# antoni-wojcik/OpenCL-Raytracing

Hardware: AMD Instinct MI355X
Metric: Msamples/sec (rays/sec) at 1920×1080, 64 spp; % HBM roofline (higher is better)
Workload: dtype f32

## Files before the change

include/rt_amd.h:

```cpp
#ifndef RT_AMD_H
#define RT_AMD_H

#include <stddef.h>
#include <stdint.h>

#ifdef __cplusplus
extern "C" {
#endif

#define RT_ABI_VERSION 3

#define RT_OK 0
#define RT_EINVAL (-1)
#define RT_ENODEVICE (-2)
#define RT_EHIP (-3)
#define RT_ESTATE (-4)
#define RT_ERANGE (-5)

#define RT_TRIANGLE_EPSILON 0.0000001f
#define RT_MIN_DISTANCE 0.001f
#define RT_MAX_DISTANCE 1000.0f
#define RT_DEPTH 30
#define RT_RANDOM_BUFFER_SIZE 100000
#define RT_RANDOM_TABLE_FLOATS (4 * RT_RANDOM_BUFFER_SIZE)
// ... 290 lines not shown
int rt_read_variance(rt_context *ctx, int which, float *out, size_t bytes);
int rt_device_variance(rt_context *ctx, int which, void **d_out);

#define RT_DENOISE_MOMENTS_MIN_COUNT 4u
int rt_read_moments(rt_context *ctx, float *m2, size_t bytes);
int rt_device_moments(rt_context *ctx, void **d_m2);
int rt_moments_merge(uint32_t nA, const float sumA[3], float m2A, uint32_t nB, const float sumB[3], float m2B, float *m2_out);
int rt_denoise_moments(rt_context *ctx, const rt_denoise_variance_params *p);

int rt_sync(rt_context *ctx);

int rt_trace_samples(rt_context *ctx, const float camera[12], const uint32_t *x, const uint32_t *y,
                     const uint32_t *sample, size_t n, float *out_rgb);


int rt_read_image(rt_context *ctx, float *rgba, size_t bytes);

int rt_read_linear(rt_context *ctx, float *rgba, size_t bytes);

int rt_device_image(rt_context *ctx, void **d_rgba);
int rt_device_accum(rt_context *ctx, void **d_rgba);

#define RT_OPT_PREFIX_SHARING 1
#define RT_OPT_MAX_THREADS_PER_LAUNCH 2
#define RT_OPT_SAMPLE_QUEUE 3
#define RT_OPT_ACCEL 4
#define RT_OPT_WALK_SLICES 5
#define RT_OPT_PREFIX_TREE 7
#define RT_OPT_WAVE_FILL 8
#define RT_OPT_PREFIX_CACHE 9
#define RT_OPT_LOOKAHEAD 10
#define RT_OPT_EXACT_GRID 11
#define RT_OPT_MOMENTS 12
#define RT_OPT_ARITH 6
#define RT_ARITH_IEEE 0
#define RT_ARITH_ROCM_OCL_NOCONTRACT 1
#define RT_ARITH_ROCM_OCL 2
int rt_set_option(rt_context *ctx, int option, int value);


int rt_enable_counters(rt_context *ctx, int enable);
int rt_reset_counters(rt_context *ctx);
int rt_get_counters(rt_context *ctx, rt_counters *out);

int rt_debug_check_accel(const rt_scene_desc *scene, uint64_t stats[8], char *err, size_t err_len);

int rt_get_debug_counters(rt_context *ctx, uint64_t out[2]);

int rt_walk_overflow(rt_context *ctx, uint32_t *flags_out);

uint64_t rt_counters_bytes(const rt_counters *c);

int rt_last_kernel_ms(rt_context *ctx, float *ms);

int rt_kernel_ms_history(rt_context *ctx, float *ms, size_t cap, size_t *n_out);

int rt_debug_hit(rt_context *ctx, int kind, const float *rays, const uint32_t *prim, const uint32_t *face, size_t n,
                 float *out12);
int rt_debug_material(rt_context *ctx, int routine, const float *in16, size_t n, float *out9);
int rt_debug_div3(rt_context *ctx, const float *in4, size_t n, float *out6);
int rt_debug_builtin(rt_context *ctx, int op, const float *in8, size_t n, float *out4);
int rt_debug_queue_sums(rt_context *ctx, const float *in3, uint32_t npix, uint32_t count, uint32_t group_log2, float *out4);

int rt_stage_ms_history(rt_context *ctx, float *first_ms, float *second_ms, size_t cap, size_t *n_out);

int rt_prefix_cache_stats(rt_context *ctx, uint64_t *hits, uint64_t *misses);

int rt_lookahead_stats(rt_context *ctx, uint64_t *batches, uint64_t *served, uint64_t *direct, uint64_t *discarded);

int rt_lookahead_plan(int width, int height, int option_value, uint32_t sample_counter, uint32_t *batch_out);

int rt_sample_units(uint32_t seg_cap, uint32_t pixels_per_unit, uint32_t count_light, uint32_t count_heavy, uint32_t *units_out);

int rt_sample_grid_stats(rt_context *ctx, uint64_t *launches, uint64_t *exact, uint64_t *workgroups, uint64_t *live_last);

int rt_debug_live_list(rt_context *ctx, uint32_t out[4]);

int rt_debug_queue_pixels(uint32_t count, uint32_t waves_per_simd, uint32_t static_float4, uint32_t granule, uint32_t *pixels_out);

typedef struct rt_sample_facts {
    uint32_t count, glog2;
    uint32_t n, seg_cap;
    uint32_t material_count, sphere_count, plane_count, lens_count, model_count;
    uint32_t sphere_bvh, mesh_bvh;
    uint32_t walk_jobs;
    uint32_t faces;
    uint32_t cu_count;
    uint32_t count_enabled, sample_queue, walk_slices, wave_fill, moments;
    uint32_t exact, count_light, count_heavy;
} rt_sample_facts;

#define RT_PLAN_FIXED 0u
#define RT_PLAN_QUEUE 1u
#define RT_PLAN_WALK 2u
#define RT_PLAN_GENERIC_COUNT 0xFFFFFFFFu

typedef struct rt_sample_plan {
    uint32_t family;
    uint32_t count, accel, geom, waves, moments, count_log2, multi;
// ... 50 lines not shown
```

opencl-raytracing_amd/_abi.py:

```python
import ctypes as C

import numpy as np

RT_ABI_VERSION = 3
DEPTH = 30
RANDOM_BUFFER_SIZE = 100000
RANDOM_TABLE_FLOATS = 4 * RANDOM_BUFFER_SIZE
MAX_DIM = 16384
MAX_SAMPLE = 65535

T_REFRACTIVE, T_REFLECTIVE, T_DIELECTRIC, T_DIFFUSE, T_TEXTURED, T_LIGHT = range(6)
MAT_NAMES = {
    "refractive": T_REFRACTIVE,
    "reflective": T_REFLECTIVE,
    "dielectric": T_DIELECTRIC,
    "diffuse": T_DIFFUSE,
    "textured": T_TEXTURED,
    "light": T_LIGHT,
}

MATERIAL = np.dtype([("type", "<i4"), ("_p0", "<i4", (3,)), ("color", "<f4", (4,)), ("extra_data", "<f4"),
                     ("_p1", "<i4", (3,))])
SPHERE = np.dtype([("pos", "<f4", (4,)), ("r", "<f4"), ("mat_ID", "<u4"), ("_p", "<u4", (2,))])
PLANE = np.dtype([("pos", "<f4", (4,)), ("normal", "<f4", (4,)), ("mat_ID", "<u4"), ("_p", "<u4", (3,))])
# ... 118 lines not shown
    _fields_ = [("iterations", C.c_uint32), ("sigma_luminance", C.c_float), ("sigma_normal", C.c_float),
                ("sigma_position", C.c_float), ("sigma_albedo", C.c_float), ("flags", C.c_uint32)]


def denoise_prototypes(lib):
    vp, sz = C.c_void_p, C.c_size_t
    lib.rt_render_features.argtypes = [vp, vp]
    lib.rt_read_features.argtypes = [vp, vp, sz]
    lib.rt_device_features.argtypes = [vp, C.POINTER(vp)]
    lib.rt_denoise.argtypes = [vp, C.POINTER(DenoiseParams)]
    lib.rt_read_denoised.argtypes = [vp, vp, sz]
    lib.rt_device_denoised.argtypes = [vp, C.POINTER(vp)]
    lib.rt_denoise_variance.argtypes = [vp, C.POINTER(DenoiseVarianceParams)]
    lib.rt_read_variance.argtypes = [vp, C.c_int, vp, sz]
    lib.rt_device_variance.argtypes = [vp, C.c_int, C.POINTER(vp)]
    lib.rt_render_features_chain.argtypes = [vp, vp, C.POINTER(FeatureChainParams)]
    lib.rt_feature_chain_signature.argtypes = [vp, C.c_uint32, C.POINTER(C.c_uint32)]


DENOISE_MOMENTS_MIN_COUNT = 4


def moments_prototypes(lib):
    vp, sz, u32, f32 = C.c_void_p, C.c_size_t, C.c_uint32, C.c_float
    f3 = C.POINTER(f32)
    lib.rt_read_moments.argtypes = [vp, vp, sz]
    lib.rt_device_moments.argtypes = [vp, C.POINTER(vp)]
    lib.rt_moments_merge.argtypes = [u32, f3, f32, u32, f3, f32, f3]
    lib.rt_denoise_moments.argtypes = [vp, C.POINTER(DenoiseVarianceParams)]


def prefix_cache_prototypes(lib):
    lib.rt_prefix_cache_stats.argtypes = [C.c_void_p, C.POINTER(C.c_uint64), C.POINTER(C.c_uint64)]


def lookahead_prototypes(lib):
    p64 = C.POINTER(C.c_uint64)
    lib.rt_lookahead_stats.argtypes = [C.c_void_p, p64, p64, p64, p64]
    lib.rt_lookahead_plan.argtypes = [C.c_int, C.c_int, C.c_int, C.c_uint32, C.POINTER(C.c_uint32)]


def sample_grid_prototypes(lib):
    p64, u32 = C.POINTER(C.c_uint64), C.c_uint32
    lib.rt_sample_units.argtypes = [u32, u32, u32, u32, C.POINTER(u32)]
    lib.rt_sample_grid_stats.argtypes = [C.c_void_p, p64, p64, p64, p64]
    lib.rt_debug_live_list.argtypes = [C.c_void_p, C.POINTER(u32)]
    lib.rt_debug_wave_fixed.argtypes = [C.c_void_p, C.POINTER(C.c_uint64)]
    lib.rt_debug_stage_block.argtypes = [C.c_void_p, C.c_void_p, C.c_size_t, C.POINTER(u32)]
    lib.rt_debug_queue_pixels.argtypes = [u32, u32, u32, u32, C.POINTER(u32)]
    lib.rt_debug_queue_occupancy.argtypes = [C.c_void_p, u32, C.POINTER(C.c_int)]
    lib.rt_debug_plan_samples.argtypes = [C.POINTER(SampleFacts), C.POINTER(SamplePlan)]
    lib.rt_debug_last_sample_plan.argtypes = [C.c_void_p, C.POINTER(SampleFacts), C.POINTER(SamplePlan)]


class _U32Record(C.Structure):

    def __init__(self, **kw):
        super().__init__(**{k: int(v) for k, v in kw.items()})

    def as_dict(self):
        return {k: int(getattr(self, k)) for k, _ in self._fields_}


class SampleFacts(_U32Record):
    _fields_ = [(k, C.c_uint32) for k in (
        "count", "glog2", "n", "seg_cap", "material_count", "sphere_count", "plane_count", "lens_count", "model_count",
# ... 289 lines not shown
```

opencl-raytracing_amd/csrc/pt_kernels.hip:

```cpp
#include <hip/hip_runtime.h>

#include <algorithm>

#include "pt_device.hpp"
#include "pt_moments.hpp"
#include "pt_chain.hpp"
#include "rt_context.hpp"
#include "pt_kernels.hpp"

#ifndef PT_GATHER_UNIT
#define PT_GATHER_UNIT 0
#endif

namespace PT_NS {
using namespace rtamd;


PT_DEV uint32_t live_take(const FrameParams &fp, const uint32_t *__restrict__ live_count, uint32_t unit, uint32_t want,
                          uint32_t &first) {
    const uint32_t cap = fp.seg_cap;
    const uint32_t cnt_l = min(live_count[0], cap);
    const uint32_t cnt_h = min(live_count[LIVE_HEAVY_COUNTER], cap - cnt_l);
    const uint32_t units_h = want ? (cnt_h + want - 1u) / want : 0u;
    const bool heavy = unit < units_h;
// ... 12 lines not shown
    for (int i = 0; i < PT_N_COUNTERS; i++) {
        uint32_t v = cn.c[i];
#pragma unroll
        for (int off = 32; off > 0; off >>= 1) v += __shfl_xor(v, off);
        if ((threadIdx.x & 63) == 0 && v) atomicAdd(&row[i], (unsigned long long)v * scale);
    }
}

PT_DEV void zero_counters(LaneCounters &cn) {
#pragma unroll
    for (int i = 0; i < PT_N_COUNTERS; i++) cn.c[i] = 0;
}

PT_DEV uint32_t lanes_below(unsigned long long m) {
    return __builtin_amdgcn_mbcnt_hi((uint32_t)(m >> 32), __builtin_amdgcn_mbcnt_lo((uint32_t)m, 0u));
}

PT_DEV V3 group_sum(V3 sum, uint32_t g) {
    for (uint32_t off = g >> 1; off > 0; off >>= 1) {
        sum.x += __shfl_xor(sum.x, off);
        sum.y += __shfl_xor(sum.y, off);
        sum.z += __shfl_xor(sum.z, off);
    }
    return sum;
}

PT_DEV void accumulate(float4 *__restrict__ accum, size_t pix, V3 sum, uint32_t count) {
    float4 a = accum[pix];
    a.x += sum.x;
    a.y += sum.y;
    a.z += sum.z;
    a.w += (float)count;
    accum[pix] = a;
}

PT_DEV void moments_update(const float4 *accum, float *m2, size_t pix, V3 sum, uint32_t count, float m2B) {
    const float4 a = accum[pix];
    m2[pix] = moments_merge(a.w, a.x, a.y, a.z, m2[pix], (float)count, sum.x, sum.y, sum.z, m2B);
}

struct LaneMoments {
    float n, m2;
};
PT_DEV void moments_fold(LaneMoments &lm, V3 sum, V3 s) {
    lm.m2 = moments_merge(lm.n, sum.x, sum.y, sum.z, lm.m2, 1.0f, s.x, s.y, s.z, 0.0f);
    lm.n += 1.0f;
}
PT_DEV V3 group_sum_moments(V3 sum, LaneMoments &lm, uint32_t g) {
    for (uint32_t off = g >> 1; off > 0; off >>= 1) {
        const V3 o = mk(__shfl_xor(sum.x, off), __shfl_xor(sum.y, off), __shfl_xor(sum.z, off));
        const float on = __shfl_xor(lm.n, off), om2 = __shfl_xor(lm.m2, off);
        lm.m2 = moments_merge(lm.n, sum.x, sum.y, sum.z, lm.m2, on, o.x, o.y, o.z, om2);
        lm.n += on;
        sum.x += o.x;
        sum.y += o.y;
        sum.z += o.z;
    }
    return sum;
}

PT_DEV V3 final_sum(V3 col, uint32_t count, uint32_t group_log2) {
    const uint32_t g = 1u << group_log2;
    V3 Y = mk(0.0f, 0.0f, 0.0f);
    for (uint32_t k = 0; k < (count >> group_log2); k++) Y = Y + col;
    V3 X = Y + col;
    uint32_t r = count & (g - 1u);
// ... 178 lines not shown

#ifndef PT_PREFIX_WAVES
#define PT_PREFIX_WAVES 4
#endif
template <bool COUNT, bool ACCEL, bool TREES = false>
__global__ __launch_bounds__(256, TREES ? PT_PREFIX_WAVES : 1) void pt_prefix(DeviceScene sc, FrameParams fp, PixelRec *__restrict__ recs,
                                                 uint32_t *__restrict__ live, uint32_t *__restrict__ live_count,
                                                 float4 *__restrict__ accum, unsigned long long *counters,
                                                 FinalPix *__restrict__ finals, uint32_t *__restrict__ final_n) {
    __shared__ float4 s_mat[PT_LDS_STATIC_FLOAT4];
    LaneCounters cn;
    if (COUNT) zero_counters(cn);
    Ctx c{sc, stage_materials(sc, s_mat), &cn};
    c.lwin = staged_winners(sc, s_mat);
    c.lpln = staged_planes(sc, s_mat);

    uint32_t slot = fp.slot_begin + blockIdx.x * 256u + threadIdx.x;
    uint32_t x = 0, y = 0;
    bool valid = slot < fp.slot_end && slot_to_pixel(fp, slot, x, y) && pixel_active(fp, x, y);
    bool is_live = false, is_final = false;
    PixelRec rec;
    rec.p_kind = rec.n_extra = rec.d = rec.out = rec.col = make_float4(0.0f, 0.0f, 0.0f, 0.0f);
    if (valid) {
        Ray r0 = primary_ray(fp.cam, x, y, fp.w, fp.h);
        rec = trace_prefix<COUNT, ACCEL>(c, r0, x, y);
    }
    if (valid) {
        bool final_px = (__float_as_uint(rec.p_kind.w) & 0xFFu) == REC_FINAL;
        if (final_px) {
            is_final = true;
            if (accum) {
                const V3 fsum = final_sum(xyz(rec.out), fp.count, fp.group_log2);
                if (fp.m2) moments_update(accum, fp.m2, (size_t)y * fp.w + x, fsum, fp.count, 0.0f);
                accumulate(accum, (size_t)y * fp.w + x, fsum, fp.count);
            }
            if (COUNT) cn.c[CN_SAMPLES] += 1;
        } else {
            is_live = true;
        }
    }
    const uint32_t lane = threadIdx.x & 63u, wv = threadIdx.x >> 6;
    const uint32_t kb = __float_as_uint(rec.p_kind.w);
    const bool lane_heavy = valid && (((kb >> 8) & 0xFFu) >= 2u || is_glass_vertex(rec));
    const bool wg_heavy = __syncthreads_or(lane_heavy ? 1 : 0) != 0;
    const bool glass = TREES && is_live && is_glass_vertex(rec);
    __shared__ uint32_t s_wave_n[4], s_wave_g[4], s_wave_f[4], s_base, s_tree0;
    __shared__ uint32_t s_tpos[256];
    __shared__ uint32_t s_wn[PT_TREE_LEVELS];
    __shared__ uint16_t s_wait[PT_TREE_LEVELS > 2 ? 2 : 1][256u << (PT_TREE_LEVELS - 1)];
    unsigned long long m = __ballot(is_live);
    const unsigned long long gm = __ballot(glass);
    const unsigned long long fm = __ballot(is_final);
    if (lane == 0) {
        s_wave_n[wv] = (uint32_t)__popcll(m);
        s_wave_f[wv] = (uint32_t)__popcll(fm);
        if (TREES) s_wave_g[wv] = (uint32_t)__popcll(gm);
    }
    __syncthreads();
    if (threadIdx.x == 0) {
        uint32_t total = s_wave_n[0] + s_wave_n[1] + s_wave_n[2] + s_wave_n[3];
        s_base = total ? atomicAdd(&live_count[wg_heavy ? LIVE_HEAVY_COUNTER : 0u], total) : 0u;
        if (TREES) {
            const uint32_t trees = s_wave_g[0] + s_wave_g[1] + s_wave_g[2] + s_wave_g[3];
            s_tree0 = trees ? atomicAdd(fp.tree_count, trees) : 0u;
            for (uint32_t l = 0; l < PT_TREE_LEVELS; l++) s_wn[l] = 0u;
        }
    }
// ... 27 lines not shown
        uint32_t before = 0;
        for (uint32_t k = 0; k < wv; k++) before += s_wave_g[k];
        const uint32_t j = before + lanes_below(gm);
        if (j < nt) {
            s_tpos[j] = pos;
            fp.trees[tree0 + j].dec[0].hsh = 0u;
        }
    }
    __syncthreads();
    for (uint32_t level = 0; level < PT_TREE_LEVELS; level++) {
        const uint32_t items = 2u * (level ? s_wn[level] : nt);
        for (uint32_t t = threadIdx.x; t < items; t += 256u) {
            const uint32_t e = level ? (uint32_t)s_wait[(level - 1u) & 1u][t >> 1] : (1u << 8) | (t >> 1);
            const uint32_t j = e & 0xFFu, heap = e >> 8, which = t & 1u, tree = tree0 + j;
            if (tree_step<ACCEL>(c, fp.trees + tree, tree, heap, which, level + 1u == PT_TREE_LEVELS, recs + s_tpos[j],
                                 fp.tree_wait + (size_t)tree * PT_TREE_WAITS)) {
                const uint32_t k = atomicAdd(&s_wn[level + 1u], 1u);
                s_wait[level & 1u][k] = (uint16_t)(((2u * heap + which) << 8) | j);
            }
        }
        if (level + 1u < PT_TREE_LEVELS) __syncthreads();
    }
}

#if !PT_GATHER_UNIT
__global__ __launch_bounds__(256) void pt_final_replay(FrameParams fp, const FinalPix *__restrict__ finals,
                                                       const uint32_t *__restrict__ final_n, float4 *__restrict__ accum) {
    if (threadIdx.x >= min(final_n[blockIdx.x], 256u)) return;
    const FinalPix e = finals[blockIdx.x * 256u + threadIdx.x];
    uint32_t x = 0, y = 0;
    if (!slot_to_pixel(fp, e.slot, x, y)) return;
    const V3 fsum = final_sum(mk(e.r, e.g, e.b), fp.count, fp.group_log2);
    if (fp.m2) moments_update(accum, fp.m2, (size_t)y * fp.w + x, fsum, fp.count, 0.0f);
    accumulate(accum, (size_t)y * fp.w + x, fsum, fp.count);
}
#endif

PT_DEV size_t ring_at(const FrameParams &fp, size_t pix, uint32_t j) {
    return PT_RING_PIXEL_MAJOR ? pix * fp.count + j : j * ((size_t)fp.w * fp.h) + pix;
}

#if !PT_GATHER_UNIT
__global__ __launch_bounds__(256) void pt_final_retrace(FrameParams fp, const FinalPix *__restrict__ finals,
                                                        const uint32_t *__restrict__ final_n) {
    if (threadIdx.x >= min(final_n[blockIdx.x], 256u)) return;
    const FinalPix e = finals[blockIdx.x * 256u + threadIdx.x];
    uint32_t x = 0, y = 0;
    if (!slot_to_pixel(fp, e.slot, x, y)) return;
    const size_t pix = (size_t)y * fp.w + x;
    const float4 at = fp.la_image[pix];
    V3 prev = mk(at.x, at.y, at.z);
    const V3 sum = mk(0.0f, 0.0f, 0.0f) + mk(e.r, e.g, e.b);
    for (uint32_t j = 0; j < fp.count; j++) {
        prev = retrace_step(prev, sum, fp.first + j);
        fp.la_ring[ring_at(fp, pix, j)] = make_float4(prev.x, prev.y, prev.z, 1.0f);
    }
}
#endif

template <bool COUNT, bool ACCEL>
__global__ __launch_bounds__(256) void pt_samples(DeviceScene sc, FrameParams fp, const PixelRec *__restrict__ recs,
                                                  const uint32_t *__restrict__ live,
                                                  const uint32_t *__restrict__ live_count,
                                                  float4 *__restrict__ accum, unsigned long long *counters) {
    __shared__ float4 s_mat[PT_LDS_STATIC_FLOAT4];
    {
        uint32_t e0 = 0;
// ... 214 lines not shown
    q.slot[3 * idx + 2] = rgb.z;
}

#ifndef PT_QUEUE_SUMS_TREE
#define PT_QUEUE_SUMS_TREE 1
#endif
PT_DEV V3 queue_lane_sum(const WaveQueue &q, uint32_t p, uint32_t l, uint32_t g) {
    V3 sum = mk(0.0f, 0.0f, 0.0f);
    const uint32_t n = p < q.npix ? q.count : 0u;
    for (uint32_t j = l; j < n; j += g) {
        const LdsF32 sl = q.slot + 3u * (p * q.count + j);
        sum = sum + mk(sl[0], sl[1], sl[2]);
    }
    return sum;
}
template <int OFF>
PT_DEV float row_add(float v) {
    return v + __int_as_float(__builtin_amdgcn_update_dpp(0, __float_as_int(v), 0x100 + OFF, 0xF, 0xF, false));
}
template <int OFF>
PT_DEV V3 row_add(V3 v) { return mk(row_add<OFF>(v.x), row_add<OFF>(v.y), row_add<OFF>(v.z)); }
PT_DEV float row_pair_add(float a, float b) {
    const auto r = __builtin_amdgcn_permlane16_swap(__float_as_uint(a), __float_as_uint(b), false, false);
    return __uint_as_float(r[0]) + __uint_as_float(r[1]);
}
PT_DEV V3 queue_lane_slot64(const WaveQueue &q, uint32_t p, uint32_t l) {
    V3 sum = mk(0.0f, 0.0f, 0.0f);
    if (p < q.npix) {
        const LdsF32 sl = q.slot + 3u * (p * 64u + l);
        sum = sum + mk(sl[0], sl[1], sl[2]);
    }
    return sum;
}
template <int CL = -1>
PT_DEV void queue_sums_tree(const WaveQueue &q, const FrameParams &fp, float4 *__restrict__ accum) {
    if (CL == 6) {
        static_assert(QUEUE_SLOTS / 64u <= 8u, "two passes of four pixels");
        const uint32_t lane = threadIdx.x, half = lane >> 5, i = lane & 31u, row = lane >> 4;
#pragma unroll
        for (uint32_t pb = 0; pb < 8u; pb += 4u) {
            if (pb >= q.npix) break;
            V3 a = queue_lane_slot64(q, pb + half, i), b = queue_lane_slot64(q, pb + 2u + half, i);
            a = a + queue_lane_slot64(q, pb + half, i + 32u);
            b = b + queue_lane_slot64(q, pb + 2u + half, i + 32u);
            V3 sum = mk(row_pair_add(a.x, b.x), row_pair_add(a.y, b.y), row_pair_add(a.z, b.z));
            sum = row_add<1>(row_add<2>(row_add<4>(row_add<8>(sum))));
            const uint32_t p = pb + ((row & 1u) << 1 | row >> 1);
            if (p < q.npix && (lane & 15u) == 0u) accumulate(accum, (size_t)q.xy[p].y * fp.w + q.xy[p].x, sum, 64u);
        }
        return;
    }
    const uint32_t lane = threadIdx.x, gl = fp.group_log2;
    if (gl >= 5u) {
        const uint32_t half = lane >> 5, i = lane & 31u, g = 1u << gl, row = lane >> 4;
        for (uint32_t pb = 0; pb < q.npix; pb += 4u) {
            V3 a = queue_lane_sum(q, pb + half, i, g), b = queue_lane_sum(q, pb + 2u + half, i, g);
            if (gl == 6u) {
                a = a + queue_lane_sum(q, pb + half, i + 32u, g);
                b = b + queue_lane_sum(q, pb + 2u + half, i + 32u, g);
            }
            V3 sum = mk(row_pair_add(a.x, b.x), row_pair_add(a.y, b.y), row_pair_add(a.z, b.z));
            sum = row_add<1>(row_add<2>(row_add<4>(row_add<8>(sum))));
            const uint32_t p = pb + ((row & 1u) << 1 | row >> 1);
            if (p < q.npix && (lane & 15u) == 0u) accumulate(accum, (size_t)q.xy[p].y * fp.w + q.xy[p].x, sum, q.count);
        }
    } else {
        const uint32_t g = 1u << gl, ppp = 64u >> gl;
        for (uint32_t pb = 0; pb < q.npix; pb += ppp) {
            const uint32_t p = pb + (lane >> gl), l = lane & (g - 1u);
            V3 sum = queue_lane_sum(q, p, l, g);
            if (gl >= 4u) sum = row_add<8>(sum);
            if (gl >= 3u) sum = row_add<4>(sum);
            if (gl >= 2u) sum = row_add<2>(sum);
            if (gl >= 1u) sum = row_add<1>(sum);
            if (p < q.npix && l == 0u) accumulate(accum, (size_t)q.xy[p].y * fp.w + q.xy[p].x, sum, q.count);
        }
    }
}
template <bool MOMENTS, bool BUTTERFLY = false, int CL = -1>
PT_DEV void queue_sums(const WaveQueue &q, const FrameParams &fp, float4 *__restrict__ accum) {
    __builtin_amdgcn_fence(__ATOMIC_SEQ_CST, "wavefront");
    __builtin_amdgcn_wave_barrier();
    if (PT_QUEUE_SUMS_TREE && !MOMENTS && !BUTTERFLY) return queue_sums_tree<CL>(q, fp, accum);
    const uint32_t lane = threadIdx.x;
    const uint32_t g = 1u << fp.group_log2, ppp = 64u >> fp.group_log2;
    for (uint32_t pb = 0; pb < q.npix; pb += ppp) {
        uint32_t p = pb + (lane >> fp.group_log2), l = lane & (g - 1u);
        V3 sum = mk(0.0f, 0.0f, 0.0f);
        if (p < q.npix)
            for (uint32_t j = l; j < q.count; j += g) {
                const LdsF32 sl = q.slot + 3u * (p * q.count + j);
                sum = sum + mk(sl[0], sl[1], sl[2]);
            }
        sum = group_sum(sum, g);
        if (MOMENTS) {
            const float mean = moments_lum(sum.x, sum.y, sum.z) / (float)q.count;
            float dev2 = 0.0f;
            if (p < q.npix)
                for (uint32_t j = l; j < q.count; j += g) {
                    const LdsF32 sl = q.slot + 3u * (p * q.count + j);
                    const float d = moments_lum(sl[0], sl[1], sl[2]) - mean;
                    dev2 += d * d;
                }
            for (uint32_t off = g >> 1; off > 0; off >>= 1) dev2 += __shfl_xor(dev2, off);
            if (p < q.npix && l == 0) moments_update(accum, fp.m2, (size_t)q.xy[p].y * fp.w + q.xy[p].x, sum, q.count, dev2);
        }
        if (p < q.npix && l == 0) accumulate(accum, (size_t)q.xy[p].y * fp.w + q.xy[p].x, sum, q.count);
    }
}

static_assert(QUEUE_MAX_PIXELS * 4u <= 64u, "queue_replay maps (pixel, channel) to the wave's lanes");
template <bool CAM = false>
PT_DEV void queue_replay(const WaveQueue &q, const FrameParams &fp) {
    static_assert(!CAM || !PT_RING_PIXEL_MAJOR, "the camera look-ahead's start image is frame 0 of a frame-major ring (one contiguous "
                                                "device copy of the image); the pixel-major A/B layout has no such frame");
    __builtin_amdgcn_fence(__ATOMIC_SEQ_CST, "wavefront");
// ... 842 lines not shown
static_assert(MODE_ACCUM == 0 && MODE_TRACE == 1 && MODE_RETRACE == 2, "render_kernel's table is indexed by the mode");
static RenderKernel render_kernel(int mode, bool count, bool accel) {
    static const RenderKernel k[3][2][2] = {
        {{pt_render<MODE_ACCUM, false, false>, pt_render<MODE_ACCUM, false, true>}, {pt_render<MODE_ACCUM, true, false>, pt_render<MODE_ACCUM, true, true>}},
        {{pt_render<MODE_TRACE, false, false>, pt_render<MODE_TRACE, false, true>}, {pt_render<MODE_TRACE, true, false>, pt_render<MODE_TRACE, true, true>}},
        {{pt_render<MODE_RETRACE, false, false>, pt_render<MODE_RETRACE, false, true>}, {pt_render<MODE_RETRACE, true, false>, pt_render<MODE_RETRACE, true, true>}}};
    return k[mode][count][accel];
}

static uint32_t slots_per_launch(const rt_context *ctx, uint32_t glog2) { return std::max(ctx->max_threads_per_launch >> glog2, 1u); }
static uint32_t range_end(uint32_t b, uint32_t slots, uint32_t per) { return slots - b > per ? b + per : slots; }

template <class Body>
static int launch_ranges(rt_context *ctx, FrameParams &fp, uint32_t slots, Body body) {
    const uint32_t per = slots_per_launch(ctx, fp.group_log2);
    hipEvent_t *evp = ctx->ev[ctx->ev_count % rt_context::EV_RING];
    HIP_TRY(ctx, hipEventRecord(evp[0], ctx->stream));
    HIP_TRY(ctx, hipEventRecord(evp[2], ctx->stream));
    for (uint32_t b = 0; b < slots; b = fp.slot_end) {
        fp.slot_begin = b;
        fp.slot_end = range_end(b, slots, per);
        const int rc = body();
        if (rc != RT_OK) return rc;
    }
    HIP_TRY(ctx, hipGetLastError());
    HIP_TRY(ctx, hipEventRecord(evp[1], ctx->stream));
    ctx->ev_count++;
    return RT_OK;
}

int launch_render(rt_context *ctx, int mode, const float cam[12], uint32_t first, uint32_t count, uint32_t glog2, float4 *accum,
                  const BlockMask *mask, float *m2) {
    if (mode < MODE_ACCUM || mode > MODE_RETRACE) return fail(ctx, RT_EINVAL, "unknown render mode %d", mode);
    FrameParams fp = frame_params(ctx, cam, first, count, glog2);
    apply_mask(fp, mask);
    fp.m2 = mode == MODE_ACCUM ? m2 : nullptr;
    const DeviceScene sc = device_scene(ctx);
    const uint32_t slots = fp.slot_end;
    if (slots == 0) return RT_OK;
    const RenderKernel kernel = render_kernel(mode, ctx->count_enabled, scene_has_accel(sc));
    return launch_ranges(ctx, fp, slots, [&]() -> int {
        const uint64_t threads = (uint64_t)(fp.slot_end - fp.slot_begin) << glog2;
        hipLaunchKernelGGL(kernel, dim3((unsigned)((threads + 255) / 256)), dim3(256), 0, ctx->stream, sc, fp, accum, ctx->image.p, ctx->counters.p);
        return RT_OK;
    });
}

using SampleFacts = rt_sample_facts;
using SamplePlan = rt_sample_plan;
using CameraFacts = rt_camera_facts;
using CameraPlan = rt_camera_plan;

struct QueueSize {
    uint32_t accel, geom, waves, pixels_per_wave, ppw_cap, lds_face_f4, static_f4, lds_bytes;
};
template <class Facts>
static QueueSize queue_size(const Facts &f, bool stage_faces) {
    QueueSize q = {};
    const bool simple_geom = f.lens_count == 0 && f.model_count == 0;
    const bool sphere_bvh_only = f.sphere_bvh && !f.mesh_bvh;
    q.accel = f.sphere_bvh || f.mesh_bvh;
    q.geom = !q.accel || sphere_bvh_only ? (simple_geom ? 0u : 1u) : 2u;
    q.waves = !q.accel ? PT_Q_WAVES : ((sphere_bvh_only && simple_geom) ? PT_Q_WAVES_SPHERE_BVH : PT_Q_WAVES_ACCEL);
    q.static_f4 = lds_static_used(f.material_count, f.sphere_count, f.plane_count);
    const uint32_t want_units = (f.cu_count ? f.cu_count : 256u) * 4u * 6u * PT_UNITS_PER_WAVE_SLOT;
    const uint32_t ppw_full = (64u + f.count - 1u) / f.count;
// ... 140 lines not shown
}

using PrefixKernel = void (*)(DeviceScene, FrameParams, PixelRec *, uint32_t *, uint32_t *, float4 *, unsigned long long *, FinalPix *, uint32_t *);
static PrefixKernel prefix_kernel(bool count, bool accel, bool trees) {
    static const PrefixKernel plain[2][2] = {{pt_prefix<false, false>, pt_prefix<false, true>}, {pt_prefix<true, false>, pt_prefix<true, true>}};
    static const PrefixKernel tree[2] = {pt_prefix<false, false, true>, pt_prefix<false, true, true>};
    return trees ? tree[accel] : plain[count][accel];
}
static void launch_first_stage(rt_context *ctx, const DeviceScene &sc, const FrameParams &fp, bool hit, bool lookahead, float4 *accum, uint32_t *live_count) {
    const rt_context::Slots &ss = ctx->slots;
    const dim3 grid(fp.seg_cap / 256u), block(256);
    if (!hit)
        hipLaunchKernelGGL(prefix_kernel(ctx->count_enabled, scene_has_accel(sc), fp.tree_cap != 0u), grid, block, 0, ctx->stream, sc, fp,
                           ss.recs.p, ss.live.p, live_count, accum, ctx->counters.p, ss.finals.p, ss.final_n.p);
    else if (!lookahead)
        hipLaunchKernelGGL(pt_final_replay, grid, block, 0, ctx->stream, fp, ss.finals.p, ss.final_n.p, accum);
    if (lookahead) hipLaunchKernelGGL(pt_final_retrace, grid, block, 0, ctx->stream, fp, ss.finals.p, ss.final_n.p);
}

static bool lookahead_ok(const rt_context *ctx, const FrameParams &fp, const float4 *accum, const BlockMask *mask, const float *m2) {
    return !accum && !m2 && !mask && !ctx->count_enabled && ctx->world == 1 && ctx->sample_queue && fp.count <= QUEUE_SLOTS &&
           (ctx->max_threads_per_launch >> fp.group_log2) >= fp.slot_end;
}

static void refresh_stage_block(rt_context *ctx, const DeviceScene &sc) {
    if (!PT_STAGE_COPY || ctx->stage_block.generation == ctx->prefix_cache.generation) return;
    if (lds_static_used(sc.material_count, sc.sphere_count, sc.plane_count))
        hipLaunchKernelGGL(pt_stage_block, dim3(1), dim3(64), 0, ctx->stream, sc,
                           reinterpret_cast<float4 *>(reinterpret_cast<char *>(ctx->materials.p) + stage_block_offset(sc.material_count)));
    ctx->stage_block.generation = ctx->prefix_cache.generation;
    ctx->stage_block.builds++;
}

static int launch_fused_any(rt_context *ctx, const float cam[12], uint32_t first, uint32_t count, uint32_t glog2, float4 *accum,
                            const BlockMask *mask, float4 *ring, float *m2) {
    FrameParams fp = frame_params(ctx, cam, first, count, glog2);
    apply_mask(fp, mask);
    fp.m2 = m2;
    if (ring) {
        if (!lookahead_ok(ctx, fp, accum, mask, m2))
            return fail(ctx, RT_EINVAL, "a look-ahead launch needs the sample queue, an unsharded frame in one slot range and no counters");
        fp.la_ring = ring;
        fp.la_image = ctx->image.p;
    }
    const DeviceScene sc = device_scene(ctx);
    const uint32_t slots = fp.slot_end;
    if (slots == 0) return RT_OK;
    int rc = ensure_slots(ctx, slots);
    if (rc) return rc;
    refresh_stage_block(ctx, sc);
    const rt_context::Slots &ss = ctx->slots;
    uint32_t *live_count = ss.live.p + ss.capacity + 256u;
    const uint32_t per = slots_per_launch(ctx, glog2);
    const bool tree_on = ctx->prefix_tree == 2 || (ctx->prefix_tree == 1 && count >= PT_TREE_MIN_SAMPLES);
    const bool keepable = !mask && !ctx->count_enabled && per >= slots;
    uint32_t cam_bits[12];
    memcpy(cam_bits, cam, sizeof cam_bits);
    const bool hit = prefix_lookup(ctx->prefix_cache, keepable, tree_on, cam_bits);
    bool exact = false;
    if ((rc = learn_live_counts(ctx, hit, live_count, &exact)) != RT_OK) return rc;
    rt_context::SampleGrid &sg = ctx->sample_grid;
    hipEvent_t *evp = ctx->ev[ctx->ev_count % rt_context::EV_RING];
    HIP_TRY(ctx, hipEventRecord(evp[0], ctx->stream));
    for (uint32_t b = 0; b < slots; b = fp.slot_end) {
        fp.slot_begin = b;
        fp.slot_end = range_end(b, slots, per);
        if (!hit) HIP_TRY(ctx, hipMemsetAsync(live_count, 0, LIVE_COUNT_STRIDE * sizeof(uint32_t), ctx->stream));
        fp.trees = ss.trees.p;
        fp.tree_wait = ss.tree_wait.p;
        fp.tree_count = live_count + LIVE_TREE_COUNTER;
        fp.tree_cap = (tree_on && !ctx->count_enabled) ? (uint32_t)ss.tree_capacity : 0u;
        fp.seg_cap = (fp.slot_end - fp.slot_begin + 255u) / 256u * 256u;
        const SampleFacts facts = sample_facts(ctx, sc, fp, exact);
        const SamplePlan plan = plan_samples(facts);
        fp.lds_face_f4 = plan.lds_face_f4;
        launch_first_stage(ctx, sc, fp, hit, ring != nullptr, accum, live_count);
        HIP_TRY(ctx, hipEventRecord(evp[2], ctx->stream));
        if ((rc = launch_plan(ctx, plan, sc, fp, accum, live_count)) != RT_OK) return rc;
        sg.last_facts = facts, sg.last_plan = plan;
        sg.launches++;
        sg.workgroups += plan.grid_units;
        if (plan.grid_units && plan.family == RT_PLAN_QUEUE && plan.count_log2 == 6u) sg.count64_launches++;
        if (exact) { sg.exact_launches++; sg.live_last = plan.grid_units; }
    }
    HIP_TRY(ctx, hipGetLastError());
    HIP_TRY(ctx, hipEventRecord(evp[1], ctx->stream));
    ctx->ev_count++;
    if (hit) ctx->prefix_cache.hits++; else ctx->prefix_cache.misses++;
    if (keepable) prefix_keep(ctx->prefix_cache, tree_on, cam_bits);
    return RT_OK;
}

int launch_fused(rt_context *ctx, const float cam[12], uint32_t first, uint32_t count, uint32_t glog2, float4 *accum, const BlockMask *mask, float *m2) {
    return launch_fused_any(ctx, cam, first, count, glog2, accum, mask, nullptr, m2);
}

int launch_lookahead(rt_context *ctx, const float cam[12], uint32_t first, uint32_t count, float4 *ring) {
    if (!ring || count < 1u) return fail(ctx, RT_EINVAL, "look-ahead launch without a ring");
    return launch_fused_any(ctx, cam, first, count, group_log2_for(count), nullptr, nullptr, ring, nullptr);
}

static RenderKernel camera_render_kernel(bool count, bool accel) {
    static const RenderKernel k[2][2] = {{pt_render<MODE_ACCUM, false, false, true>, pt_render<MODE_ACCUM, false, true, true>},
                                         {pt_render<MODE_ACCUM, true, false, true>, pt_render<MODE_ACCUM, true, true, true>}};
    return k[count][accel];
}
typedef void (*RayRenderKernel)(DeviceScene, FrameParams, float4 *, unsigned long long *);
static RayRenderKernel ray_render_kernel(bool count, bool accel, bool sets) {
    static const RayRenderKernel k[2][2] = {{pt_render_rays<false, false>, pt_render_rays<false, true>},
                                            {pt_render_rays<true, false>, pt_render_rays<true, true>}};
    static const RayRenderKernel k_sets[2][2] = {{pt_render_raysets<false, false>, pt_render_raysets<false, true>},
// ... 1 lines not shown
    return sets ? k_sets[count][accel] : k[count][accel];
}
static const pt::GatherKernels &gather_kernels() {
#if PT_ARITH == 0
    return *pt::gather_kernels_a0();
#elif PT_ARITH == 1
    return *pt::gather_kernels_a1();
#else
    return *pt::gather_kernels_a2();
#endif
}

struct SampleSource {
    bool rays, hemi;
    const void *p;
    size_t n;
    uint32_t set_size;
    const float *cam0;
};

static int launch_source(rt_context *ctx, const SampleSource &src, uint32_t first, uint32_t count, uint32_t glog2, float4 *accum,
                         const BlockMask *mask, float *m2, float4 *ring) {
    const bool sets = src.set_size != 0u && !src.hemi;
    if (!src.rays) {
        if (!src.p || count < 1u || count > RT_SPP_PER_LAUNCH) return fail(ctx, RT_EINVAL, "a camera launch takes 1 .. %u blocks", RT_SPP_PER_LAUNCH);
    } else {
        if (!src.p || !accum || src.n < 1u || src.n > (1u << 28) || count < 1u || count > RT_SPP_PER_LAUNCH)
            return fail(ctx, RT_EINVAL, "a ray launch takes 1 .. 2^28 rays and 1 .. %u samples", RT_SPP_PER_LAUNCH);
        if (src.set_size > RT_RAY_SET_MAX || (uint64_t)src.n * src.set_size > (1ull << 31))
            return fail(ctx, RT_EINVAL, "a ray-set launch takes sets of 1 .. %u records, 2^31 records in all", RT_RAY_SET_MAX);
        if (mask && src.n != (size_t)ctx->width * ctx->height)
            return fail(ctx, RT_EINVAL, "a masked ray launch takes one ray per pixel of the %d x %d frame", ctx->width, ctx->height);
    }
    FrameParams fp = src.rays ? frame_params(ctx, src.cam0, first, count, glog2, 0, 1)
                              : frame_params(ctx, src.cam0, first, count, glog2);
    apply_mask(fp, mask);
    fp.m2 = m2;
    if (src.rays) fp.rays = reinterpret_cast<const float4 *>(src.p);
    else fp.cams = reinterpret_cast<const float *>(src.p);
    const DeviceScene sc = device_scene(ctx);
    if (ring) {
        if (src.rays || !lookahead_ok(ctx, fp, accum, mask, m2) || plan_camera_samples(camera_facts(ctx, sc, fp)).family != RT_CAMERA_PLAN_QUEUE)
            return fail(ctx, RT_EINVAL, "a look-ahead launch needs the sample queue, an unsharded frame in one slot range and no counters");
        fp.la_ring = ring;
    }
    const uint32_t slots = src.rays ? (uint32_t)src.n : fp.slot_end;
    if (slots == 0) return RT_OK;
    refresh_stage_block(ctx, sc);
    return launch_ranges(ctx, fp, slots, [&]() -> int {
        const CameraFacts facts = camera_facts(ctx, sc, fp);
        const CameraPlan plan = plan_camera_samples(facts);
        const dim3 grid(plan.grid_units), block(plan.block_size);
        fp.lds_face_f4 = plan.lds_face_f4;
        if (plan.family == RT_CAMERA_PLAN_QUEUE) {
            const QueueRow *r = find_queue_row(ctx, src.rays ? "ray" : "camera", plan.accel, plan.geom, plan.waves);
            if (!r) return RT_ESTATE;
            const QueueKernel kernel = !src.rays ? r->cams[ring != nullptr] : src.hemi ? gather_kernels().queue(plan.accel, plan.geom, plan.waves)
                                       : sets ? r->ray_sets : r->rays;
            if (!kernel) return fail(ctx, RT_ESTATE, "no pt_samples_q_hemi for the plan (accel %u, geom %u, %u waves)", plan.accel, plan.geom, plan.waves);
            hipLaunchKernelGGL(kernel, grid, block, plan.lds_bytes, ctx->stream,
                               sc, fp, (const PixelRec *)nullptr, (const uint32_t *)nullptr, (const uint32_t *)nullptr, accum,
                               ctx->counters.p, plan.pixels_per_wave);
        } else if (src.rays) {
            hipLaunchKernelGGL(src.hemi ? gather_kernels().fixed(plan.count != 0u, plan.accel != 0u) : ray_render_kernel(plan.count != 0u, plan.accel != 0u, sets),
                               grid, block, 0, ctx->stream, sc, fp, accum, ctx->counters.p);
        } else {
// ... 218 lines not shown
```

opencl-raytracing_amd/csrc/pt_samples_q_kernel.hpp:

```cpp
#if PT_Q_LOOKAHEAD_FORM == 4
template <bool ACCEL, int GEOM, int WAVES>
__global__ __launch_bounds__(64, WAVES) void pt_samples_q_hemi(DeviceScene sc, FrameParams fp, const PixelRec *__restrict__ recs,
                                                         const uint32_t *__restrict__ live,
                                                         const uint32_t *__restrict__ live_count,
                                                         float4 *__restrict__ accum, unsigned long long *counters,
                                                         uint32_t pixels_per_wave) {
    constexpr bool COUNT = false, MOMENTS = false, CAM = true, CAM_LA = false, RAYS = true, SETS = false, HEMI = true;
    constexpr int COUNT_LOG2 = -1;
#elif PT_Q_LOOKAHEAD_FORM == 3
template <bool ACCEL, int GEOM, int WAVES>
__global__ __launch_bounds__(64, WAVES) void pt_samples_q_raysets(DeviceScene sc, FrameParams fp, const PixelRec *__restrict__ recs,
                                                            const uint32_t *__restrict__ live,
                                                            const uint32_t *__restrict__ live_count,
                                                            float4 *__restrict__ accum, unsigned long long *counters,
                                                            uint32_t pixels_per_wave) {
    constexpr bool COUNT = false, MOMENTS = false, CAM = true, CAM_LA = false, RAYS = true, SETS = true, HEMI = false;
    constexpr int COUNT_LOG2 = -1;
#elif PT_Q_LOOKAHEAD_FORM == 2
template <bool ACCEL, int GEOM, int WAVES>
__global__ __launch_bounds__(64, WAVES) void pt_samples_q_rays(DeviceScene sc, FrameParams fp, const PixelRec *__restrict__ recs,
                                                         const uint32_t *__restrict__ live,
                                                         const uint32_t *__restrict__ live_count,
                                                         float4 *__restrict__ accum, unsigned long long *counters,
                                                         uint32_t pixels_per_wave) {
// ... 181 lines not shown
                hn = h.n;
                hmat = h.mat;
                int type;
                float extra;
                load_material<BY_COUNT>(c, h.mat, type, extra, col);
                if (BY_USE) htype = (uint32_t)type;
                if (type == RT_LIGHT) {
                    if (SIP_HIT) out = vmin<MIN_FAST>(out, col);
                    else res = vmin<MIN_FAST>(out, col);
                    done = true;
                } else if (type == RT_TEXTURED) {
                    if (COUNT) cn.c[CN_N_TEXFETCH]++;
                    float tu = h.u, tv = h.v;
                    if (PT_TEXEL_LAZY && GEOM == 0 && !COUNT && !ACCEL) asm("" : "+v"(tu), "+v"(tv));
                    col = texture_rgb(c.sc, tu, tv, h.tex);
                }
            }
            if (done) {
                queue_put(q, idx, SIP_HIT ? out : res);
                active = false;
            } else if (PT_RNG_PREFETCH == 2) {
                rnd = fetch_rnd_b(sc.table, r.d, depth, bv, bu);
            }
        }
        PT_STAMP(c, 4);
    }
#if PT_STAMPS
    if (threadIdx.x == 0 && q.npix)
        for (int k = 0; k < 6; k++) atomicAdd(&counters[(size_t)COUNTER_REPLICAS * COUNTER_STRIDE + k], c.st[k]);
#endif
    static_assert(!CAM_LA || (CAM && ACCEL), "the look-ahead kernels of the camera entry's ACCEL rows");
    constexpr bool LA_BRANCH = CAM ? !ACCEL : !COUNT && !MOMENTS;
    if (CAM_LA || (!RAYS && LA_BRANCH && fp.la_ring)) queue_replay<CAM>(q, fp);
    else queue_sums<MOMENTS, COUNT || ACCEL, COUNT_LOG2>(q, fp, accum);
    flush_counters<COUNT>(cn, counters, 1);
}
```

opencl-raytracing_amd/csrc/pt_types.hpp:

```cpp
#pragma once
#include <hip/hip_runtime.h>
#include <stdint.h>

#include "../../include/rt_amd.h"

namespace pt {

#define PT_DEV __device__ __forceinline__
#define PT_HD __host__ __device__ inline

#define PT_LDS_MATERIALS 64
#define PT_LDS_WINNERS 64
#define PT_SPHERE_BATCH 4

struct DeviceScene {
    const rt_material *materials;
    const rt_sphere *spheres;
    const float4 *sph4;
    const rt_plane *planes;
    const rt_lens *lenses;
    const rt_float3 *vertices;
    const rt_float2 *uvs;
    const uint32_t *indices;
    const rt_mesh *meshes;
    const rt_model *models;
    const float *table;
    const float4 *tex;
    int tex_w, tex_h, tex_layers;
    float tex_wf, tex_hf;
    uint32_t material_count, sphere_count, sphere_batches, plane_count, lens_count, model_count;
    const float4 *faces;
    const uint32_t *mesh_face_base;
    const float4 *mbvh_nodes;
    const float4 *mbvh_faces;
// ... 51 lines not shown
#define PT_TREE_LEVELS 2
#endif
#define PT_TREE_DECISIONS ((1 << PT_TREE_LEVELS) - 1)
#define PT_TREE_LEAVES (1 << PT_TREE_LEVELS)
struct TreeDecision {
    uint32_t hsh;
    float prob;
    uint32_t depth;
    uint16_t child[2];
};
struct PixelTree {
    TreeDecision dec[PT_TREE_DECISIONS + 1];
    PixelRec leaf[PT_TREE_LEAVES];
};
#define PT_TREE_WAITS (PT_TREE_LEAVES - 2)

enum RenderMode { MODE_ACCUM = 0, MODE_TRACE = 1, MODE_RETRACE = 2 };

#ifndef PT_RING_PIXEL_MAJOR
#define PT_RING_PIXEL_MAJOR 0
#endif

struct FrameParams {
    float cam[12];
    int w, h;
    int tile_w_log2, tile_h_log2;
    uint32_t tiles_x, tiles_total;
    uint32_t rank, world;
    uint32_t slot_begin, slot_end;
    uint32_t first, count;
    uint32_t group_log2;
    uint32_t seg_cap;
    float inv_count;
    PixelTree *trees;
    PixelRec *tree_wait;
    uint32_t *tree_count;
    uint32_t tree_cap;
    uint32_t lds_face_f4;
    const uint32_t *block_active;
    uint32_t blk_w_log2, blk_h_log2, blocks_x;
    float4 *la_ring;
    union {
        const float4 *la_image;
        const float *cams;
        const float4 *rays;
        const float4 *feats;
    };
    float *m2;
};

struct BlockMask {
    const uint32_t *active;
    uint32_t w_log2, h_log2, blocks_x;
};

#define LIVE_COUNT_STRIDE 32u
#define LIVE_TREE_COUNTER 16u
#define LIVE_HEAVY_COUNTER 24u

#define COUNTER_REPLICAS 512
#define COUNTER_STRIDE 16

PT_DEV bool slot_to_pixel(const FrameParams &fp, uint32_t slot, uint32_t &x, uint32_t &y) {
    uint32_t tpix_log2 = fp.tile_w_log2 + fp.tile_h_log2;
    uint32_t k = slot >> tpix_log2, in = slot & ((1u << tpix_log2) - 1u);
    uint32_t t = fp.rank + k * fp.world;
    if (t >= fp.tiles_total) return false;
    uint32_t tx = t % fp.tiles_x, ty = t / fp.tiles_x;
    x = (tx << fp.tile_w_log2) + (in & ((1u << fp.tile_w_log2) - 1u));
    y = (ty << fp.tile_h_log2) + (in >> fp.tile_w_log2);
    return x < (uint32_t)fp.w && y < (uint32_t)fp.h;
}

PT_DEV bool pixel_active(const FrameParams &fp, uint32_t x, uint32_t y) {
    return !fp.block_active || fp.block_active[(y >> fp.blk_h_log2) * fp.blocks_x + (x >> fp.blk_w_log2)] != 0u;
}

PT_DEV bool ray_active(const FrameParams &fp, uint32_t index) {
    if (!fp.block_active) return true;
    const uint32_t y = index / (uint32_t)fp.w, x = index - y * (uint32_t)fp.w;
    return fp.block_active[(y >> fp.blk_h_log2) * fp.blocks_x + (x >> fp.blk_w_log2)] != 0u;
}
// ... 9 lines not shown
```

opencl-raytracing_amd/csrc/rt_amd.hip:

```cpp
#include <hip/hip_runtime.h>

#include <algorithm>
#include <cmath>
#include <cfloat>
#include <cstdarg>
#include <cstdio>
#include <cstdlib>
#include <cstring>
#include <functional>
#include <mutex>
#include <new>
#include <string>
#include <vector>

#include "rt_context.hpp"
#include "pt_kernels.hpp"
#include "pt_moments.hpp"
#include "pt_chain.hpp"
#include "scene_prep.hpp"

using namespace pt;
using namespace rtamd;
using namespace scene_prep;

// ... 236 lines not shown
    rt_context::Lookahead &la = ctx->lookahead;
    la.discarded += la.pending;
    la.pending = 0;
}

void lookahead_validate(rt_context *ctx) {
    const rt_context::Lookahead &la = ctx->lookahead;
    if (la.pending && (la.key_generation != ctx->prefix_cache.generation || la.key_epoch != ctx->image_epoch ||
                       la.next_sample != ctx->sample_counter + 1u))
        lookahead_drop(ctx);
}

int alloc_frame(rt_context *ctx, int w, int h) {
    ctx->slots = {};
    ctx->prefix_changed();
    ctx->image_epoch++;
    lookahead_drop(ctx);
    ctx->lookahead.ring = {};
    ctx->lookahead.ring_frames = 0;
    ctx->lookahead.ring_failed = false;
    ctx->adaptive = {};
    ctx->features = {};
    ctx->denoise = {};
    ctx->moments.m2 = {};
    ctx->moments.valid = false;
    const size_t px = (size_t)w * h;
    HIP_TRY(ctx, ctx->image.alloc(px));
    HIP_TRY(ctx, ctx->accum.alloc(px));
    HIP_TRY(ctx, hipMemset(ctx->image.p, 0, px * sizeof(float4)));
    HIP_TRY(ctx, hipMemset(ctx->accum.p, 0, px * sizeof(float4)));
    ctx->width = w;
    ctx->height = h;
    ctx->accum_count = 0;
    ctx->sample_counter = 0;
    return RT_OK;
}

int check_ready(rt_context *ctx, const float *cam) {
    if (!ctx) return RT_EINVAL;
    if (!cam) return fail(ctx, RT_EINVAL, "camera block is NULL");
    if (!ctx->have_scene) return fail(ctx, RT_ESTATE, "no scene: call rt_set_scene first");
    if (ctx->scene_uses_textures && (ctx->tex_layers <= 0 || ctx->max_texture_id >= (uint32_t)ctx->tex_layers))
        return fail(ctx, RT_ERANGE, "scene has textured meshes (max texture id %u) but only %d texture layers are set",
                    ctx->max_texture_id, ctx->tex_layers);
    return RT_OK;
}

}

namespace rtamd {
int read_back(rt_context *ctx, void *dst, size_t bytes, const void *src, size_t need, const char *what, bool ready,
              const char *producer) {
    if (!dst || bytes != need) return fail(ctx, RT_EINVAL, "%s buffer must be %zu bytes", what, need);
    if (!ready) return fail(ctx, RT_ESTATE, "no %s call since the frame was (re)allocated", producer);
    HIP_TRY(ctx, hipSetDevice(ctx->device));
    HIP_TRY(ctx, hipMemcpyAsync(dst, src, need, hipMemcpyDeviceToHost, ctx->stream));
    HIP_TRY(ctx, hipStreamSynchronize(ctx->stream));
    return RT_OK;
}
}

namespace {

int apply_arith(rt_context *ctx) {
    const bool w_is_radius = ctx->arith == RT_ARITH_ROCM_OCL;
    auto rec = [&](const rt_sphere &s) {
        volatile float r2 = s.r * s.r;
        return make_float4(s.pos.x, s.pos.y, s.pos.z, w_is_radius ? s.r : (float)r2);
    };
    const uint32_t n = (uint32_t)ctx->h_spheres.size();
    const uint32_t batches = (n + PT_SPHERE_BATCH - 1) / PT_SPHERE_BATCH;
    std::vector<float4> v((size_t)(batches + 1) * PT_SPHERE_BATCH, make_float4(0.0f, 0.0f, 0.0f, w_is_radius ? NAN : -INFINITY));
    for (uint32_t i = 0; i < n; i++) v[i] = rec(ctx->h_spheres[i]);
    HIP_TRY(ctx, ctx->sph4.upload(v.data(), v.size()));
    ctx->sphere_batches = batches;
    if (!ctx->h_bvh_idx.empty()) {
        std::vector<float4> leaf(ctx->h_bvh_idx.size());
        for (size_t i = 0; i < leaf.size(); i++) leaf[i] = rec(ctx->h_spheres[ctx->h_bvh_idx[i]]);
        HIP_TRY(ctx, ctx->bvh_sph.upload(leaf.data(), leaf.size()));
    }
    HIP_TRY(ctx, ctx->faces.upload(ctx->h_faces.data(), ctx->h_faces.size()));
    HIP_TRY(ctx, ctx->mbvh_faces.upload(ctx->h_mbvh_faces.data(), ctx->h_mbvh_faces.size()));
    if (ctx->arith != RT_ARITH_IEEE) {
        int rc = ctx->ks->launch_face_normals(ctx, ctx->faces.p, (uint32_t)(ctx->h_faces.size() / 3));
        if (rc == RT_OK) rc = ctx->ks->launch_face_normals(ctx, ctx->mbvh_faces.p, (uint32_t)(ctx->h_mbvh_faces.size() / 3));
        if (rc != RT_OK) return rc;
        HIP_TRY(ctx, hipStreamSynchronize(ctx->stream));
    }
    return RT_OK;
}

}


extern "C" {

int rt_abi_version(void) { return RT_ABI_VERSION; }

const char *rt_last_error(const rt_context *ctx) {
    if (ctx) return ctx->error.c_str();
    std::lock_guard<std::mutex> lk(g_err_mutex);
    return g_create_error.c_str();
}

int rt_make_random_table(uint64_t seed, float *out, size_t n) {
    if (!out || n != RT_RANDOM_TABLE_FLOATS) return fail(nullptr, RT_EINVAL, "table must hold %d floats", RT_RANDOM_TABLE_FLOATS);
    make_table(seed, out);
    return RT_OK;
}

int rt_create(int device, int width, int height, rt_context **out) {
    if (!out) return fail(nullptr, RT_EINVAL, "out is NULL");
    *out = nullptr;
    if (width < 1 || height < 1 || width > RT_MAX_DIM || height > RT_MAX_DIM)
        return fail(nullptr, RT_EINVAL, "frame size %dx%d outside 1..%d", width, height, RT_MAX_DIM);
    int n = 0;
    if (hipGetDeviceCount(&n) != hipSuccess || n < 1)
        return fail(nullptr, RT_ENODEVICE, "no HIP device visible (this library has no CPU path)");
    if (device < 0 || device >= n) return fail(nullptr, RT_ENODEVICE, "device %d out of range (%d visible)", device, n);
    hipDeviceProp_t prop;
// ... 30 lines not shown
    if (const char *e = getenv("RT_PREFIX_CACHE")) ctx->prefix_cache.enabled = strcmp(e, "0") != 0;
    if (const char *e = getenv("RT_LOOKAHEAD")) { if (strcmp(e, "0") == 0) ctx->lookahead.k = 0; }
    if (const char *e = getenv("RT_EXACT_GRID")) ctx->sample_grid.exact = strcmp(e, "0") != 0;
    if (hipHostMalloc((void **)&ctx->sample_grid.h_counts, LIVE_COUNT_STRIDE * sizeof(uint32_t), hipHostMallocDefault) != hipSuccess ||
        hipEventCreateWithFlags(&ctx->sample_grid.counts_ev, hipEventDisableTiming) != hipSuccess) { ctx->error = "live-count read-back allocation failed"; return bail(RT_EHIP); }
    if ((rc = alloc_frame(ctx, width, height)) != RT_OK) return bail(rc);
    if ((rc = rt_set_seed(ctx, 0xC0FFEEull)) != RT_OK) return bail(rc);
    if ((rc = rt_set_textures(ctx, nullptr, 0, 0, 0)) != RT_OK) return bail(rc);
    *out = ctx;
    return RT_OK;
}

void rt_destroy(rt_context *ctx) {
    if (!ctx) return;
    (void)hipSetDevice(ctx->device);
    if (ctx->own_stream) (void)hipStreamSynchronize(ctx->own_stream);
    for (int i = 0; i < rt_context::EV_RING; i++)
        for (int k = 0; k < 3; k++)
            if (ctx->ev[i][k]) (void)hipEventDestroy(ctx->ev[i][k]);
    if (ctx->sample_grid.counts_ev) (void)hipEventDestroy(ctx->sample_grid.counts_ev);
    if (ctx->sample_grid.h_counts) (void)hipHostFree(ctx->sample_grid.h_counts);
    for (hipEvent_t e : ctx->cameras.read)
        if (e) (void)hipEventDestroy(e);
    if (ctx->cameras.h_table) (void)hipHostFree(ctx->cameras.h_table);
    if (ctx->own_stream) (void)hipStreamDestroy(ctx->own_stream);
    delete ctx;
}

int rt_resize(rt_context *ctx, int width, int height) {
    if (!ctx) return RT_EINVAL;
    if (width < 1 || height < 1 || width > RT_MAX_DIM || height > RT_MAX_DIM)
        return fail(ctx, RT_EINVAL, "frame size %dx%d outside 1..%d", width, height, RT_MAX_DIM);
    HIP_TRY(ctx, hipSetDevice(ctx->device));
    HIP_TRY(ctx, hipStreamSynchronize(ctx->stream));
    return alloc_frame(ctx, width, height);
}

int rt_set_stream(rt_context *ctx, void *hip_stream) {
    if (!ctx) return RT_EINVAL;
    HIP_TRY(ctx, hipSetDevice(ctx->device));
    HIP_TRY(ctx, hipStreamSynchronize(ctx->stream));
    ctx->stream = hip_stream ? (hipStream_t)hip_stream : ctx->own_stream;
    ctx->prefix_changed();
    ctx->ev_count = 0;
    return RT_OK;
}

int rt_set_scene(rt_context *ctx, const rt_scene_desc *d) {
    if (!ctx) return RT_EINVAL;
    if (!d) return fail(ctx, RT_EINVAL, "scene is NULL");
    ctx->prefix_changed();
    {
        PreparedScene ps;
        std::string err;
        if (int rc = prepare_scene(*d, ps, err)) return fail(ctx, rc, "%s", err.c_str());
        HIP_TRY(ctx, hipSetDevice(ctx->device));
        HIP_TRY(ctx, hipStreamSynchronize(ctx->stream));
        ctx->have_scene = false;
        HIP_TRY(ctx, ctx->materials.upload(d->materials, d->material_count,
                                           lds_static_used(d->material_count, d->sphere_count, d->plane_count) * sizeof(float4)));
        ctx->stage_block.generation = ~0ull;
        HIP_TRY(ctx, ctx->spheres.upload(d->spheres, d->sphere_count));
        ctx->h_spheres.assign(d->spheres, d->spheres + d->sphere_count);
        HIP_TRY(ctx, ctx->mesh_face_base.upload(ps.face_base.data(), ps.face_base.size()));
        HIP_TRY(ctx, ctx->mbvh_nodes.upload(ps.mesh_packed.data(), ps.mesh_packed.size()));
        ctx->have_mesh_bvh = ps.have_mesh_bvh;
        HIP_TRY(ctx, ctx->mbvh_face_idx.upload(ps.leaf_face_idx.data(), ps.leaf_face_idx.size()));
        HIP_TRY(ctx, ctx->mesh_bvh_root.upload(ps.mesh_roots.data(), ps.mesh_roots.size()));
        ctx->walk_jobs.release();
        if (!ps.walk_jobs.empty()) HIP_TRY(ctx, ctx->walk_jobs.upload(ps.walk_jobs.data(), ps.walk_jobs.size()));
        ctx->bvh_node_count = ps.bvh_node_count;
        if (!ps.sphere_nodes.empty()) {
            HIP_TRY(ctx, ctx->bvh_nodes.upload(ps.sphere_boxes.data(), ps.sphere_boxes.size()));
            HIP_TRY(ctx, ctx->bvh_links.upload(ps.sphere_links.data(), ps.sphere_links.size()));
            HIP_TRY(ctx, ctx->bvh_idx.upload(ps.sphere_leaf_idx.data(), ps.sphere_leaf_idx.size()));
            ctx->bvh_rmax = ps.bvh_rmax;
            for (int k = 0; k < 3; k++) { ctx->bvh_lo[k] = ps.bvh_lo[k]; ctx->bvh_hi[k] = ps.bvh_hi[k]; }
        }
        HIP_TRY(ctx, ctx->planes.upload(d->planes, d->plane_count));
        HIP_TRY(ctx, ctx->lenses.upload(d->lenses, d->lens_count));
        HIP_TRY(ctx, ctx->vertices.upload(d->vertices, d->vertex_count));
        if (d->uv_count) HIP_TRY(ctx, ctx->uvs.upload(d->uvs, d->uv_count));
        else {
            std::vector<rt_float2> zeros(d->vertex_count ? d->vertex_count : 1, rt_float2{0.0f, 0.0f});
            HIP_TRY(ctx, ctx->uvs.upload(zeros.data(), d->vertex_count));
        }
        HIP_TRY(ctx, ctx->indices.upload(d->indices, d->index_count));
        HIP_TRY(ctx, ctx->meshes.upload(d->meshes, d->mesh_count));
        HIP_TRY(ctx, ctx->models.upload(d->models, d->model_count));
        ctx->scene_uses_textures = ps.uses_tex;
        ctx->max_texture_id = ps.max_tex;
        ctx->h_bvh_idx.swap(ps.sphere_leaf_idx);
        ctx->h_faces.swap(ps.faces);
        ctx->h_mbvh_faces.swap(ps.leaf_faces);
    }
    if (int rc = apply_arith(ctx)) return rc;
    ctx->have_scene = true;
    ctx->sample_counter = 0;
    return RT_OK;
}

int rt_set_textures(rt_context *ctx, const float *rgba, int w, int h, int layers) {
    if (!ctx) return RT_EINVAL;
    ctx->prefix_changed();
    HIP_TRY(ctx, hipSetDevice(ctx->device));
    HIP_TRY(ctx, hipStreamSynchronize(ctx->stream));
    if (layers == 0) {
        float4 zero = make_float4(0.0f, 0.0f, 0.0f, 0.0f);
        HIP_TRY(ctx, ctx->tex.upload(&zero, 1));
        ctx->tex_w = ctx->tex_h = 1;
        ctx->tex_layers = 0;
        return RT_OK;
    }
    if (!rgba || w < 1 || h < 1 || layers < 1 || w > 32768 || h > 32768 || layers > 2048)
        return fail(ctx, RT_EINVAL, "bad texture array %dx%dx%d", w, h, layers);
    HIP_TRY(ctx, ctx->tex.upload((const float4 *)rgba, (size_t)w * h * layers));
    ctx->tex_w = w;
    ctx->tex_h = h;
    ctx->tex_layers = layers;
    return RT_OK;
}

int rt_set_random_table(rt_context *ctx, const float *table, size_t n) {
    if (!ctx) return RT_EINVAL;
    if (!table || n != RT_RANDOM_TABLE_FLOATS) return fail(ctx, RT_EINVAL, "table must hold %d floats", RT_RANDOM_TABLE_FLOATS);
    ctx->prefix_changed();
    HIP_TRY(ctx, hipSetDevice(ctx->device));
    HIP_TRY(ctx, hipStreamSynchronize(ctx->stream));
    HIP_TRY(ctx, ctx->table.upload(table, n));
    return RT_OK;
}

int rt_set_seed(rt_context *ctx, uint64_t seed) {
    if (!ctx) return RT_EINVAL;
    std::vector<float> t(RT_RANDOM_TABLE_FLOATS);
    make_table(seed, t.data());
    return rt_set_random_table(ctx, t.data(), t.size());
}

int rt_get_random_table(rt_context *ctx, float *out, size_t n) {
    if (!ctx) return RT_EINVAL;
    if (!out || n != RT_RANDOM_TABLE_FLOATS) return fail(ctx, RT_EINVAL, "table must hold %d floats", RT_RANDOM_TABLE_FLOATS);
    HIP_TRY(ctx, hipSetDevice(ctx->device));
    HIP_TRY(ctx, hipStreamSynchronize(ctx->stream));
    HIP_TRY(ctx, hipMemcpy(out, ctx->table.p, n * sizeof(float), hipMemcpyDeviceToHost));
    return RT_OK;
}

int rt_set_shard(rt_context *ctx, int rank, int world, int tile_w, int tile_h) {
    if (!ctx) return RT_EINVAL;
    auto log2_exact = [](int v) { int l = 0; while ((1 << l) < v) l++; return (1 << l) == v ? l : -1; };
    int lw = log2_exact(tile_w), lh = log2_exact(tile_h);
    if (world < 1 || rank < 0 || rank >= world) return fail(ctx, RT_EINVAL, "rank %d of %d", rank, world);
    if (world > 1 && ctx->moments.on) return fail(ctx, RT_EINVAL, "RT_OPT_MOMENTS is 1: sample moments are kept on unsharded contexts only");
    if (tile_w < 1 || tile_h < 1 || lw < 0 || lh < 0 || lw + lh > 16)
        return fail(ctx, RT_EINVAL, "tile %dx%d: sides must be powers of two, area <= 65536", tile_w, tile_h);
    ctx->prefix_changed();
    ctx->rank = rank;
    ctx->world = world;
    ctx->tile_w_log2 = lw;
    ctx->tile_h_log2 = lh;
    return RT_OK;
}

extern "C++" {
namespace {

#if PT_RING_PIXEL_MAJOR
__global__ __launch_bounds__(256) void pt_ring_handout(const float4 *__restrict__ ring, float4 *__restrict__ image, size_t n,
                                                       uint32_t frames, uint32_t j) {
    const size_t i = (size_t)blockIdx.x * 256u + threadIdx.x;
    if (i < n) image[i] = ring[i * frames + j];
}
#endif

uint32_t lookahead_frames(int w, int h, int k, uint32_t sample_counter) {
    if (k < 2 || sample_counter >= RT_MAX_SAMPLE) return 0u;
// ... 38 lines not shown
    la.pending = la.batch_frames = kp;
    la.next_frame = 0;
    la.next_sample = ctx->sample_counter + 1u;
    la.key_generation = ctx->prefix_cache.generation;
    la.key_epoch = ctx->image_epoch;
    la.key_is_table = table;
}

int lookahead_hand_out(rt_context *ctx, bool timed) {
    rt_context::Lookahead &la = ctx->lookahead;
    const size_t frame_px = (size_t)ctx->width * ctx->height;
    hipEvent_t *evp = ctx->ev[ctx->ev_count % rt_context::EV_RING];
    if (!timed) {
        HIP_TRY(ctx, hipEventRecord(evp[0], ctx->stream));
        HIP_TRY(ctx, hipEventRecord(evp[2], ctx->stream));
    }
#if PT_RING_PIXEL_MAJOR
    hipLaunchKernelGGL(pt_ring_handout, dim3((unsigned)((frame_px + 255) / 256)), dim3(256), 0, ctx->stream, la.ring.p, ctx->image.p,
                       frame_px, la.batch_frames, la.next_frame);
    HIP_TRY(ctx, hipGetLastError());
#else
    HIP_TRY(ctx, hipMemcpyAsync(ctx->image.p, la.ring.p + (size_t)la.next_frame * frame_px, frame_px * sizeof(float4),
                                hipMemcpyDeviceToDevice, ctx->stream));
#endif
    if (!timed) {
        HIP_TRY(ctx, hipEventRecord(evp[1], ctx->stream));
        ctx->ev_count++;
    }
    la.pending--;
    la.next_frame++;
    la.next_sample++;
    la.served++;
    ctx->sample_counter++;
    HIP_TRY(ctx, hipStreamSynchronize(ctx->stream));
    return RT_OK;
}

void remember_camera(rt_context *ctx, const float camera[12]) {
    memcpy(ctx->lookahead.last_cam, camera, sizeof ctx->lookahead.last_cam);
    ctx->lookahead.have_last_cam = true;
}

}
}

int rt_lookahead_plan(int width, int height, int option_value, uint32_t sample_counter, uint32_t *batch_out) {
    if (!batch_out) return fail(nullptr, RT_EINVAL, "batch_out is NULL");
    *batch_out = 0;
    if (width < 1 || height < 1 || width > RT_MAX_DIM || height > RT_MAX_DIM)
        return fail(nullptr, RT_EINVAL, "frame size %dx%d outside 1..%d", width, height, RT_MAX_DIM);
    if (option_value < 0 || option_value == 1 || option_value > RT_LOOKAHEAD_MAX)
        return fail(nullptr, RT_EINVAL, "RT_OPT_LOOKAHEAD takes 0 or 2..%d", RT_LOOKAHEAD_MAX);
    *batch_out = lookahead_frames(width, height, option_value, sample_counter);
    return RT_OK;
}

int rt_lookahead_stats(rt_context *ctx, uint64_t *batches, uint64_t *served, uint64_t *direct, uint64_t *discarded) {
    if (!ctx || !batches || !served || !direct || !discarded) return RT_EINVAL;
    lookahead_validate(ctx);
    *batches = ctx->lookahead.batches;
    *served = ctx->lookahead.served;
    *direct = ctx->lookahead.direct;
    *discarded = ctx->lookahead.discarded;
    return RT_OK;
}

int rt_render(rt_context *ctx, const float camera[12]) {
    int rc = check_ready(ctx, camera);
    if (rc) return rc;
    HIP_TRY(ctx, hipSetDevice(ctx->device));
    ctx->image_epoch++;
    lookahead_drop(ctx);
    remember_camera(ctx, camera);
    ctx->sample_counter = 0;
    if ((rc = ctx->ks->launch_render(ctx, MODE_TRACE, camera, 0, 1, 0, ctx->accum.p, nullptr, nullptr)) != RT_OK) return rc;
    HIP_TRY(ctx, hipStreamSynchronize(ctx->stream));
    return RT_OK;
}

int rt_render_again(rt_context *ctx, const float camera[12]) {
    int rc = check_ready(ctx, camera);
    if (rc) return rc;
    if (ctx->sample_counter >= RT_MAX_SAMPLE) return fail(ctx, RT_EINVAL, "sample counter limit %u reached", RT_MAX_SAMPLE);
    HIP_TRY(ctx, hipSetDevice(ctx->device));
    rt_context::Lookahead &la = ctx->lookahead;
    uint32_t cam_bits[12];
    memcpy(cam_bits, camera, sizeof cam_bits);
    lookahead_validate(ctx);
    if (la.pending && (la.key_is_table || memcmp(la.key_cam, cam_bits, sizeof cam_bits) != 0)) lookahead_drop(ctx);
    la.have_last_table = false;
    bool timed = false;
    if (!la.pending) {
        const uint32_t kp = lookahead_batch(ctx, cam_bits);
        if (kp) {
            if ((rc = ctx->ks->launch_lookahead(ctx, camera, ctx->sample_counter + 1u, kp, la.ring.p)) != RT_OK) return rc;
            timed = true;
            lookahead_begin(ctx, kp, false);
            memcpy(la.key_cam, cam_bits, sizeof cam_bits);
        }
    }
    remember_camera(ctx, camera);
    if (la.pending) return lookahead_hand_out(ctx, timed);
    ctx->image_epoch++;
    la.direct++;
    ctx->sample_counter++;
    if ((rc = ctx->ks->launch_render(ctx, MODE_RETRACE, camera, ctx->sample_counter, 1, 0, ctx->accum.p, nullptr, nullptr)) != RT_OK) return rc;
    HIP_TRY(ctx, hipStreamSynchronize(ctx->stream));
    return RT_OK;
}

int rt_sample_counter(const rt_context *ctx, uint32_t *out) {
    if (!ctx || !out) return RT_EINVAL;
    *out = ctx->sample_counter;
    return RT_OK;
}

extern "C++" {
namespace {
int moments_begin(rt_context *ctx) {
    rt_context::Moments &mo = ctx->moments;
    if (!mo.on) return RT_OK;
    const size_t px = (size_t)ctx->width * ctx->height;
    mo.valid = false;
    if (!mo.m2.p) HIP_TRY(ctx, mo.m2.alloc(px));
    HIP_TRY(ctx, hipMemsetAsync(mo.m2.p, 0, px * sizeof(float), ctx->stream));
    mo.valid = true;
    return RT_OK;
}

int launch_camera_samples(rt_context *ctx, const float camera[12], uint32_t first, uint32_t c, float4 *target, const BlockMask *mask, float *m2) {
    return ctx->prefix_sharing ? ctx->ks->launch_fused(ctx, camera, first, c, group_log2_for(c), target, mask, m2)
                               : ctx->ks->launch_render(ctx, MODE_ACCUM, camera, first, c, group_log2_for(c), target, mask, m2);
}

template <class Launch>
int for_each_launch(uint32_t n_samples, Launch launch) {
    for (uint32_t done = 0; done < n_samples;) {
        const uint32_t c = n_samples - done < RT_SPP_PER_LAUNCH ? n_samples - done : RT_SPP_PER_LAUNCH;
        const int rc = launch(done, c);
        if (rc != RT_OK) return rc;
        done += c;
    }
    return RT_OK;
}
}
}

int rt_clear(rt_context *ctx) {
    if (!ctx) return RT_EINVAL;
    HIP_TRY(ctx, hipSetDevice(ctx->device));
    HIP_TRY(ctx, hipMemsetAsync(ctx->accum.p, 0, (size_t)ctx->width * ctx->height * sizeof(float4), ctx->stream));
    ctx->accum_count = 0;
    return moments_begin(ctx);
}

int rt_render_spp(rt_context *ctx, const float camera[12], uint32_t first_sample, uint32_t n_samples) {
    int rc = check_ready(ctx, camera);
    if (rc) return rc;
    if (n_samples == 0) return RT_OK;
    if ((uint64_t)first_sample + n_samples - 1 > RT_MAX_SAMPLE)
        return fail(ctx, RT_EINVAL, "samples %u..+%u exceed the limit %u", first_sample, n_samples, RT_MAX_SAMPLE);
    HIP_TRY(ctx, hipSetDevice(ctx->device));
    return for_each_launch(n_samples, [&](uint32_t done, uint32_t c) {
        const int r = launch_camera_samples(ctx, camera, first_sample + done, c, ctx->accum.p, nullptr, ctx->moments.target());
        if (r == RT_OK) ctx->accum_count += c;
        return r;
    });
}

extern "C++" {
namespace {
int ensure_cameras(rt_context *ctx) {
    rt_context::Cameras &cm = ctx->cameras;
    if (cm.table.p) return RT_OK;
    const size_t floats = (size_t)rt_context::Cameras::RING * RT_SPP_PER_LAUNCH * 12u;
    if (!cm.h_table) HIP_TRY(ctx, hipHostMalloc((void **)&cm.h_table, floats * sizeof(float), hipHostMallocDefault));
    for (hipEvent_t &e : cm.read)
        if (!e) HIP_TRY(ctx, hipEventCreateWithFlags(&e, hipEventDisableTiming));
    HIP_TRY(ctx, cm.table.alloc(floats));
    return RT_OK;
}

struct CameraTable {
    uint32_t k;
// ... 150 lines not shown
    const size_t words = (size_t)n_cameras * 12u;
    const bool same = la.have_last_table && la.last_table.size() == words && memcmp(la.last_table.data(), cameras, words * sizeof(uint32_t)) == 0;
    lookahead_validate(ctx);
    if (la.pending && (!la.key_is_table || !same)) lookahead_drop(ctx);
    bool timed = false;
    if (!la.pending && same) {
        const uint32_t kp = lookahead_batch_any(ctx, true);
        if (kp) {
            if ((rc = ensure_cameras(ctx)) != RT_OK) return rc;
            std::vector<float> blocks((size_t)kp * 12u);
            for (uint32_t j = 0; j < kp; j++) memcpy(&blocks[12u * j], cameras + 12u * (size_t)((s + j) % n_cameras), 12u * sizeof(float));
            HIP_TRY(ctx, hipMemcpyAsync(la.ring.p, ctx->image.p, (size_t)ctx->width * ctx->height * sizeof(float4), hipMemcpyDeviceToDevice, ctx->stream));
            CameraTable tb;
            if ((rc = camera_table_send(ctx, blocks.data(), kp, &tb)) != RT_OK) return rc;
            rc = ctx->ks->launch_cameras(ctx, tb.d, tb.h, s, kp, group_log2_for(kp), nullptr, nullptr, nullptr, la.ring.p);
            const int rd = camera_table_read(ctx, tb);
            if (rd != RT_OK) return rd;
            if (rc != RT_OK) return rc;
            timed = true;
            lookahead_begin(ctx, kp, true);
        }
    }
    if (!same) {
        la.last_table.resize(words);
        memcpy(la.last_table.data(), cameras, words * sizeof(uint32_t));
        la.have_last_table = true;
    }
    la.have_last_cam = false;
    if (la.pending) return lookahead_hand_out(ctx, timed);
    ctx->image_epoch++;
    la.direct++;
    ctx->sample_counter++;
    if ((rc = ctx->ks->launch_render(ctx, MODE_RETRACE, cameras + 12u * (size_t)(s % n_cameras), ctx->sample_counter, 1, 0, ctx->accum.p, nullptr, nullptr)) != RT_OK) return rc;
    HIP_TRY(ctx, hipStreamSynchronize(ctx->stream));
    return RT_OK;
}

static int resolve_into(rt_context *ctx, int linear_only) {
    uint32_t n = (uint32_t)ctx->width * ctx->height;
    hipLaunchKernelGGL(pt_resolve, dim3((n + 255) / 256), dim3(256), 0, ctx->stream, ctx->accum.p, ctx->image.p, n,
                       linear_only);
    HIP_TRY(ctx, hipGetLastError());
    return RT_OK;
}

int rt_resolve(rt_context *ctx) {
    if (!ctx) return RT_EINVAL;
    HIP_TRY(ctx, hipSetDevice(ctx->device));
    ctx->image_epoch++;
    return resolve_into(ctx, 0);
}


extern "C++" {
namespace {

int ensure_adaptive(rt_context *ctx, size_t blocks) {
    rt_context::Adaptive &a = ctx->adaptive;
    if (a.scratch.p && blocks <= a.block_capacity) return RT_OK;
    a = {};
    const size_t px = (size_t)ctx->width * ctx->height;
    hipError_t e = a.scratch.alloc(px);
    if (e == hipSuccess) e = a.block_active.alloc(blocks);
    if (e == hipSuccess) e = a.block_err.alloc(blocks);
    if (e == hipSuccess) e = a.stats.alloc(PT_MERGE_REPLICAS * PT_MERGE_STRIDE);
    if (e != hipSuccess) {
        a = {};
        return fail(ctx, RT_EHIP, "adaptive buffers: %s", hipGetErrorString(e));
    }
    a.block_capacity = blocks;
    return RT_OK;
}
// ... 21 lines not shown
        return fail(ctx, RT_EINVAL, "batch %u outside 1..%u", p->batch, RT_SPP_PER_LAUNCH);
    if (rule == RULE_VARIANCE) {
        if (p->min_spp < std::max(p->batch, 2u) || p->min_spp % p->batch)
            return fail(ctx, RT_EINVAL, "min_spp %u must be a multiple of batch %u, at least it and at least 2", p->min_spp, p->batch);
    } else if (p->min_spp < 2 * p->batch || p->min_spp % p->batch)
        return fail(ctx, RT_EINVAL, "min_spp %u must be a multiple of batch %u and at least twice it", p->min_spp, p->batch);
    if (p->max_spp < p->min_spp || p->max_spp > RT_MAX_SAMPLE + 1u)
        return fail(ctx, RT_EINVAL, "max_spp %u outside min_spp %u .. %u", p->max_spp, p->min_spp, RT_MAX_SAMPLE + 1u);
    if (!(p->threshold >= 0.0f) || !std::isfinite(p->threshold))
        return fail(ctx, RT_EINVAL, "threshold must be finite and >= 0");
    *bwl = log2_pow2(p->block_w), *bhl = log2_pow2(p->block_h);
    if (p->block_w < 1 || p->block_h < 1 || p->block_w > 256 || p->block_h > 256 || *bwl < 0 || *bhl < 0)
        return fail(ctx, RT_EINVAL, "block %ux%u: sides must be powers of two in 1..256", p->block_w, p->block_h);
    return RT_OK;
}

template <class LaunchRound>
int adaptive_rounds(rt_context *ctx, AdaptiveRule rule, const rt_adaptive_params *p, int bwl, int bhl, rt_adaptive_stats *out,
                    LaunchRound launch_round) {
    int rc;
    const uint32_t bx = ((uint32_t)ctx->width + p->block_w - 1) >> bwl, by = ((uint32_t)ctx->height + p->block_h - 1) >> bhl;
    const uint32_t blocks = bx * by;
    if ((rc = ensure_adaptive(ctx, blocks)) != RT_OK) return rc;
    rt_context::Adaptive &a = ctx->adaptive;
    a.blocks = 0;
    a.variance = false;
    const size_t px = (size_t)ctx->width * ctx->height;
    if (rule == RULE_DAMMERTZ && !a.half.p) HIP_TRY(ctx, a.half.alloc(px));
    if (rule == RULE_VARIANCE && !a.pixel_err.p) HIP_TRY(ctx, a.pixel_err.alloc(px));
    const bool mom = ctx->moments.on;
    if (mom && !a.m2_scratch.p) HIP_TRY(ctx, a.m2_scratch.alloc(px));
    ctx->image_epoch++;
    const size_t bytes = px * sizeof(float4);
    HIP_TRY(ctx, hipMemsetAsync(ctx->accum.p, 0, bytes, ctx->stream));
    HIP_TRY(ctx, hipMemsetAsync(a.scratch.p, 0, bytes, ctx->stream));
    if (rule == RULE_DAMMERTZ) HIP_TRY(ctx, hipMemsetAsync(a.half.p, 0, bytes, ctx->stream));
    else HIP_TRY(ctx, hipMemsetAsync(a.pixel_err.p, 0, bytes / 4, ctx->stream));
    HIP_TRY(ctx, hipMemsetAsync(a.block_active.p, 0xFF, blocks * sizeof(uint32_t), ctx->stream));
    HIP_TRY(ctx, hipMemsetAsync(a.block_err.p, 0, blocks * sizeof(float), ctx->stream));
    ctx->accum_count = 0;
    if ((rc = moments_begin(ctx)) != RT_OK) return rc;
    if (mom) HIP_TRY(ctx, hipMemsetAsync(a.m2_scratch.p, 0, bytes / 4, ctx->stream));
    float *const m2 = mom ? ctx->moments.m2.p : nullptr, *const m2_scratch = mom ? a.m2_scratch.p : nullptr;
    const BlockMask mask{a.block_active.p, (uint32_t)bwl, (uint32_t)bhl, bx};
    MergeParams mp;
    mp.w = (uint32_t)ctx->width;
    mp.h = (uint32_t)ctx->height;
    mp.bw_log2 = (uint32_t)bwl;
    mp.bh_log2 = (uint32_t)bhl;
    mp.blocks_x = bx;
    mp.blocks = blocks;
    mp.min_spp = p->min_spp;
    mp.max_spp = p->max_spp;
    mp.threshold = p->threshold;
    uint32_t rounds = 0;
    uint64_t at_max = 0, pixel_samples = 0;
    std::vector<unsigned long long> st(PT_MERGE_REPLICAS * PT_MERGE_STRIDE);
    const size_t st_bytes = st.size() * sizeof(unsigned long long);
    for (uint32_t k = 0;; k++) {
        const uint32_t first = k * p->batch;
        const uint32_t c = std::min(p->batch, p->max_spp - first);
        if ((rc = launch_round(first, c, a.scratch.p, &mask, m2_scratch)) != RT_OK) return rc;
        mp.round = k;
        mp.count = first + c;
        HIP_TRY(ctx, hipMemsetAsync(a.stats.p, 0, st_bytes, ctx->stream));
        const dim3 grid((blocks + PT_MERGE_WAVES - 1) / PT_MERGE_WAVES), wg(64 * PT_MERGE_WAVES);
        if (rule == RULE_DAMMERTZ)
            hipLaunchKernelGGL(pt_adaptive_merge, grid, wg, 0, ctx->stream, mp, ctx->accum.p, a.half.p, a.scratch.p, a.block_active.p,
                               a.block_err.p, a.stats.p, m2, m2_scratch);
        else
            hipLaunchKernelGGL(pt_adaptive_merge_variance, grid, wg, 0, ctx->stream, mp, ctx->accum.p, a.scratch.p, a.block_active.p,
                               a.block_err.p, a.stats.p, m2, m2_scratch, a.pixel_err.p);
        HIP_TRY(ctx, hipGetLastError());
        rounds++;
        ctx->accum_count = first + c;
        HIP_TRY(ctx, hipMemcpyAsync(st.data(), a.stats.p, st_bytes, hipMemcpyDeviceToHost, ctx->stream));
        HIP_TRY(ctx, hipStreamSynchronize(ctx->stream));
        uint64_t still = 0;
        for (uint32_t r = 0; r < PT_MERGE_REPLICAS; r++) {
            still += st[r * PT_MERGE_STRIDE];
            at_max += st[r * PT_MERGE_STRIDE + 1];
            pixel_samples += st[r * PT_MERGE_STRIDE + 2];
        }
        if (still == 0) break;
    }
    if ((rc = resolve_into(ctx, 0)) != RT_OK) return rc;
    HIP_TRY(ctx, hipStreamSynchronize(ctx->stream));
    a.blocks = blocks;
    a.variance = rule == RULE_VARIANCE;
    out->rounds = rounds;
    out->pixel_samples = pixel_samples;
    out->blocks = blocks;
    out->blocks_at_max = (uint32_t)at_max;
    return RT_OK;
}

}
}

extern "C++" {
namespace {

int render_adaptive(rt_context *ctx, AdaptiveRule rule, const float camera[12], const rt_adaptive_params *p, rt_adaptive_stats *out) {
    int rc = check_ready(ctx, camera), bwl = 0, bhl = 0;
    if (rc) return rc;
    if ((rc = check_adaptive(ctx, rule, p, out, &bwl, &bhl)) != RT_OK) return rc;
    HIP_TRY(ctx, hipSetDevice(ctx->device));
    return adaptive_rounds(ctx, rule, p, bwl, bhl, out, [&](uint32_t first, uint32_t c, float4 *scratch, const BlockMask *mask, float *m2_scratch) {
        return launch_camera_samples(ctx, camera, first, c, scratch, mask, m2_scratch);
    });
}

int render_adaptive_cameras(rt_context *ctx, AdaptiveRule rule, const float *cameras, uint32_t n_cameras, const rt_adaptive_params *p,
                            rt_adaptive_stats *out) {
    int rc = check_ready(ctx, cameras), bwl = 0, bhl = 0;
    if (rc) return rc;
    if ((rc = check_adaptive(ctx, rule, p, out, &bwl, &bhl)) != RT_OK) return rc;
    if (n_cameras != p->max_spp)
        return fail(ctx, RT_EINVAL, "%u camera blocks for max_spp %u: block j is the camera of sample j", n_cameras, p->max_spp);
    HIP_TRY(ctx, hipSetDevice(ctx->device));
// ... 29 lines not shown
    return render_adaptive(ctx, RULE_DAMMERTZ, camera, p, out);
}

int rt_render_adaptive_cameras(rt_context *ctx, const float *cameras, uint32_t n_cameras, const rt_adaptive_params *p,
                               rt_adaptive_stats *out) {
    return render_adaptive_cameras(ctx, RULE_DAMMERTZ, cameras, n_cameras, p, out);
}

int rt_render_adaptive_variance(rt_context *ctx, const float camera[12], const rt_adaptive_params *p, rt_adaptive_stats *out) {
    return render_adaptive(ctx, RULE_VARIANCE, camera, p, out);
}

int rt_render_adaptive_variance_cameras(rt_context *ctx, const float *cameras, uint32_t n_cameras, const rt_adaptive_params *p,
                                        rt_adaptive_stats *out) {
    return render_adaptive_cameras(ctx, RULE_VARIANCE, cameras, n_cameras, p, out);
}

int rt_render_adaptive_rays(rt_context *ctx, const void *d_rays, size_t n_rays, uint32_t set_size, const rt_adaptive_params *p,
                            rt_adaptive_stats *out) {
    return render_adaptive_rays(ctx, RULE_DAMMERTZ, d_rays, n_rays, set_size, p, out);
}

int rt_render_adaptive_variance_rays(rt_context *ctx, const void *d_rays, size_t n_rays, uint32_t set_size, const rt_adaptive_params *p,
                                     rt_adaptive_stats *out) {
    return render_adaptive_rays(ctx, RULE_VARIANCE, d_rays, n_rays, set_size, p, out);
}

int rt_read_sample_counts(rt_context *ctx, uint32_t *counts, size_t bytes) {
    if (!ctx) return RT_EINVAL;
    const size_t n = (size_t)ctx->width * ctx->height;
    if (!counts || bytes != n * sizeof(uint32_t)) return fail(ctx, RT_EINVAL, "count buffer must be %zu bytes", n * sizeof(uint32_t));
    HIP_TRY(ctx, hipSetDevice(ctx->device));
    std::vector<float4> h(n);
    HIP_TRY(ctx, hipMemcpyAsync(h.data(), ctx->accum.p, n * sizeof(float4), hipMemcpyDeviceToHost, ctx->stream));
    HIP_TRY(ctx, hipStreamSynchronize(ctx->stream));
    for (size_t i = 0; i < n; i++) counts[i] = (uint32_t)h[i].w;
    return RT_OK;
}

int rt_read_block_error(rt_context *ctx, float *err, size_t bytes) {
    if (!ctx) return RT_EINVAL;
    const rt_context::Adaptive &a = ctx->adaptive;
    if (!a.blocks) return fail(ctx, RT_ESTATE, "no rt_render_adaptive call since the frame was (re)allocated");
    return read_back(ctx, err, bytes, a.block_err.p, a.blocks * sizeof(float), "block error");
}

int rt_read_pixel_error(rt_context *ctx, float *err, size_t bytes) {
    if (!ctx) return RT_EINVAL;
    const rt_context::Adaptive &a = ctx->adaptive;
    const size_t need = (size_t)ctx->width * ctx->height * sizeof(float);
    if (!err || bytes != need) return fail(ctx, RT_EINVAL, "pixel error buffer must be %zu bytes", need);
    if (!a.blocks || !a.variance)
        return fail(ctx, RT_ESTATE, "the last adaptive call on this frame was not rt_render_adaptive_variance(_cameras)");
    return read_back(ctx, err, bytes, a.pixel_err.p, need, "pixel error");
}

int rt_device_pixel_error(rt_context *ctx, void **d_err) {
    if (!ctx || !d_err) return RT_EINVAL;
    const rt_context::Adaptive &a = ctx->adaptive;
    if (!a.blocks || !a.variance)
        return fail(ctx, RT_ESTATE, "the last adaptive call on this frame was not rt_render_adaptive_variance(_cameras)");
    *d_err = a.pixel_err.p;
    return RT_OK;
}


}

// ... 143 lines not shown
                                                  group_log2_for(c), accum, m2);
        if (r == RT_OK && !d_accum) ctx->accum_count += c;
        return r;
    });
}

int rt_device_alloc(rt_context *ctx, size_t bytes, void **d_out) {
    if (!ctx) return RT_EINVAL;
    if (!d_out || bytes == 0) return fail(ctx, RT_EINVAL, "rt_device_alloc takes a size above 0 and a place for the pointer");
    HIP_TRY(ctx, hipSetDevice(ctx->device));
    *d_out = nullptr;
    if (hipMalloc(d_out, bytes) != hipSuccess) {
        (void)hipGetLastError();
        *d_out = nullptr;
        return fail(ctx, RT_EHIP, "no device memory for %zu bytes", bytes);
    }
    return RT_OK;
}

int rt_device_free(rt_context *ctx, void *d_ptr) {
    if (!ctx) return RT_EINVAL;
    if (!d_ptr) return RT_OK;
    HIP_TRY(ctx, hipSetDevice(ctx->device));
    HIP_TRY(ctx, hipFree(d_ptr));
    return RT_OK;
}

int rt_device_copy(rt_context *ctx, void *dst, const void *src, size_t bytes, int to_device) {
    if (!ctx) return RT_EINVAL;
    if (!dst || !src) return fail(ctx, RT_EINVAL, "rt_device_copy: a NULL pointer");
    if (bytes == 0) return RT_OK;
    HIP_TRY(ctx, hipSetDevice(ctx->device));
    HIP_TRY(ctx, hipMemcpyAsync(dst, src, bytes, to_device ? hipMemcpyHostToDevice : hipMemcpyDeviceToHost, ctx->stream));
    HIP_TRY(ctx, hipStreamSynchronize(ctx->stream));
    return RT_OK;
}

int rt_render_features_cameras(rt_context *ctx, const float *cameras, uint32_t n_cameras, const rt_feature_chain_params *p) {
    const int rc = check_ready(ctx, cameras);
    if (rc) return rc;
    const rt_feature_chain_params first_hits = {0u, 0u};
    if (!p) p = &first_hits;
    const int ok = n_cameras < 1u || n_cameras > RT_FEATURE_CAMERAS_MAX
                       ? fail(ctx, RT_EINVAL, "%u camera blocks outside 1..%u", n_cameras, RT_FEATURE_CAMERAS_MAX)
                       : check_chain_params(ctx, p);
    const int done = render_features_with(ctx, cameras, ok, [&](const FrameParams &fp, const DeviceScene &sc, rt_feature *out) {
        rt_context::Features &f = ctx->features;
        const size_t pixels = (size_t)ctx->width * ctx->height;
        if (!f.coverage.p) HIP_TRY(ctx, f.coverage.alloc(pixels));
        int r = ensure_cameras(ctx);
        if (r != RT_OK) return r;
        CameraTable tb;
        if ((r = camera_table_send(ctx, cameras, n_cameras, &tb)) != RT_OK) return r;
        r = ctx->ks->launch_features_cameras(ctx, fp, sc, tb.d, n_cameras, p->follow, p->max_chain, out,
                                             reinterpret_cast<uint2 *>(f.coverage.p));
        if (r == RT_OK) {
            hipLaunchKernelGGL(pt_features_cameras_finish, dim3((uint32_t)((pixels + 255u) / 256u)), dim3(256), 0, ctx->stream,
                               reinterpret_cast<float4 *>(out), f.coverage.p, (uint32_t)pixels, n_cameras);
            const hipError_t e = hipGetLastError();
            if (e != hipSuccess) r = fail(ctx, RT_EHIP, "pt_features_cameras_finish: %s", hipGetErrorString(e));
        }
        const int rd = camera_table_read(ctx, tb);
        return rd != RT_OK ? rd : r;
    });
    if (done == RT_OK) ctx->features.coverage_ready = true;
    return done;
}
// ... 40 lines not shown
}

int rt_device_features(rt_context *ctx, void **d_features) {
    if (!ctx || !d_features) return RT_EINVAL;
    if (!ctx->features.ready) return fail(ctx, RT_ESTATE, "no rt_render_features call since the frame was (re)allocated");
    *d_features = ctx->features.records.p;
    return RT_OK;
}

int rt_read_moments(rt_context *ctx, float *m2, size_t bytes) {
    if (!ctx) return RT_EINVAL;
    const size_t need = (size_t)ctx->width * ctx->height * sizeof(float);
    if (!m2 || bytes != need) return fail(ctx, RT_EINVAL, "moment buffer must be %zu bytes", need);
    if (!ctx->moments.target()) return fail(ctx, RT_ESTATE, "the sample moments are not valid: set RT_OPT_MOMENTS to 1, then rt_clear or rt_render_adaptive");
    return read_back(ctx, m2, bytes, ctx->moments.m2.p, need, "moment");
}

int rt_device_moments(rt_context *ctx, void **d_m2) {
    if (!ctx || !d_m2) return RT_EINVAL;
    if (!ctx->moments.target()) return fail(ctx, RT_ESTATE, "the sample moments are not valid: set RT_OPT_MOMENTS to 1, then rt_clear or rt_render_adaptive");
    *d_m2 = ctx->moments.m2.p;
    return RT_OK;
}

int rt_moments_merge(uint32_t nA, const float sumA[3], float m2A, uint32_t nB, const float sumB[3], float m2B, float *m2_out) {
    if (!sumA || !sumB || !m2_out) return fail(nullptr, RT_EINVAL, "rt_moments_merge: a pointer is NULL");
    *m2_out = moments_merge((float)nA, sumA[0], sumA[1], sumA[2], m2A, (float)nB, sumB[0], sumB[1], sumB[2], m2B);
    return RT_OK;
}

int rt_sync(rt_context *ctx) {
    if (!ctx) return RT_EINVAL;
    HIP_TRY(ctx, hipSetDevice(ctx->device));
    HIP_TRY(ctx, hipStreamSynchronize(ctx->stream));
    return RT_OK;
}

int rt_trace_samples(rt_context *ctx, const float camera[12], const uint32_t *x, const uint32_t *y,
                     const uint32_t *sample, size_t n, float *out_rgb) {
    int rc = check_ready(ctx, camera);
    if (rc) return rc;
    if (n == 0) return RT_OK;
    if (!x || !y || !sample || !out_rgb || n > (1u << 28)) return fail(ctx, RT_EINVAL, "bad probe arrays");
    for (size_t i = 0; i < n; i++)
        if (x[i] >= (uint32_t)ctx->width || y[i] >= (uint32_t)ctx->height || sample[i] > RT_MAX_SAMPLE)
            return fail(ctx, RT_EINVAL, "probe %zu (%u,%u,%u) outside the frame / sample range", i, x[i], y[i], sample[i]);
    HIP_TRY(ctx, hipSetDevice(ctx->device));
    DevBuf<uint32_t> d_in;
    DevBuf<float> d_out;
    HIP_TRY(ctx, d_in.alloc(3 * n));
    HIP_TRY(ctx, d_out.alloc(3 * n));
    HIP_TRY(ctx, hipMemcpyAsync(d_in.p, x, n * 4, hipMemcpyHostToDevice, ctx->stream));
    HIP_TRY(ctx, hipMemcpyAsync(d_in.p + n, y, n * 4, hipMemcpyHostToDevice, ctx->stream));
    HIP_TRY(ctx, hipMemcpyAsync(d_in.p + 2 * n, sample, n * 4, hipMemcpyHostToDevice, ctx->stream));
    const FrameParams fp = frame_params(ctx, camera, 0, 1, 0);
    if ((rc = ctx->ks->launch_probe(ctx, fp, device_scene(ctx), d_in.p, (uint32_t)n, d_out.p)) != RT_OK) return rc;
    HIP_TRY(ctx, hipMemcpyAsync(out_rgb, d_out.p, 3 * n * sizeof(float), hipMemcpyDeviceToHost, ctx->stream));
    HIP_TRY(ctx, hipStreamSynchronize(ctx->stream));
    return RT_OK;
}

int rt_read_image(rt_context *ctx, float *rgba, size_t bytes) {
    if (!ctx) return RT_EINVAL;
    return read_back(ctx, rgba, bytes, ctx->image.p, (size_t)ctx->width * ctx->height * sizeof(float4), "image");
}

int rt_read_linear(rt_context *ctx, float *rgba, size_t bytes) {
    if (!ctx) return RT_EINVAL;
    const size_t n = (size_t)ctx->width * ctx->height;
    if (!rgba || bytes != n * sizeof(float4)) return fail(ctx, RT_EINVAL, "image buffer must be %zu bytes", n * sizeof(float4));
    HIP_TRY(ctx, hipSetDevice(ctx->device));
    DevBuf<float4> tmp;
    HIP_TRY(ctx, tmp.alloc(n));
    hipLaunchKernelGGL(pt_resolve, dim3((n + 255) / 256), dim3(256), 0, ctx->stream, ctx->accum.p, tmp.p, (uint32_t)n, 1);
    HIP_TRY(ctx, hipGetLastError());
    HIP_TRY(ctx, hipMemcpyAsync(rgba, tmp.p, bytes, hipMemcpyDeviceToHost, ctx->stream));
    HIP_TRY(ctx, hipStreamSynchronize(ctx->stream));
    return RT_OK;
}

int rt_device_image(rt_context *ctx, void **d_rgba) {
    if (!ctx || !d_rgba) return RT_EINVAL;
    *d_rgba = ctx->image.p;
    return RT_OK;
}

int rt_device_accum(rt_context *ctx, void **d_rgba) {
    if (!ctx || !d_rgba) return RT_EINVAL;
    *d_rgba = ctx->accum.p;
    return RT_OK;
}

int rt_enable_counters(rt_context *ctx, int enable) {
    if (!ctx) return RT_EINVAL;
    ctx->count_enabled = enable != 0;
    ctx->prefix_changed();
    return RT_OK;
}

int rt_debug_check_accel(const rt_scene_desc *d, uint64_t stats[8], char *err, size_t err_len) {
    if (!d || !stats) return RT_EINVAL;
    memset(stats, 0, 8 * sizeof(uint64_t));
    PreparedScene ps;
    std::string msg;
    int rc = prepare_scene(*d, ps, msg);
    if (rc == RT_OK) rc = check_prepared(*d, ps, stats, msg);
    if (rc != RT_OK && err && err_len) snprintf(err, err_len, "%s", msg.c_str());
    return rc;
}

extern "C++" {
namespace {
template <class F>
int debug_roundtrip(rt_context *ctx, const void *in, size_t bytes, void *out, size_t out_bytes, F launch) {
    DevBuf<uint8_t> d_in, d_out;
    HIP_TRY(ctx, d_in.alloc(bytes ? bytes : 16));
    HIP_TRY(ctx, d_out.alloc(out_bytes ? out_bytes : 16));
    HIP_TRY(ctx, hipMemcpyAsync(d_in.p, in, bytes, hipMemcpyHostToDevice, ctx->stream));
    if (int rc = launch(d_in.p, d_out.p)) return rc;
    HIP_TRY(ctx, hipMemcpyAsync(out, d_out.p, out_bytes, hipMemcpyDeviceToHost, ctx->stream));
    HIP_TRY(ctx, hipStreamSynchronize(ctx->stream));
    return RT_OK;
}
}
}

int rt_debug_hit(rt_context *ctx, int kind, const float *rays, const uint32_t *prim, const uint32_t *face, size_t n,
                 float *out12) {
    if (!ctx) return RT_EINVAL;
    if (!ctx->have_scene) return fail(ctx, RT_ESTATE, "no scene: call rt_set_scene first");
    if (n == 0) return RT_OK;
    if (!rays || !out12 || kind < 0 || kind > 4 || n > (1u << 26) || (kind != 3 && !prim) || (kind == 4 && !face))
        return fail(ctx, RT_EINVAL, "bad unit-probe arguments");
    const size_t counts[5] = {ctx->spheres.n, ctx->planes.n, ctx->lenses.n, 0, ctx->meshes.n};
    std::vector<uint32_t> pf(2 * n, 0u);
    for (size_t i = 0; i < n; i++) {
        if (kind != 3) {
            if (prim[i] >= counts[kind]) return fail(ctx, RT_ERANGE, "unit probe %zu: primitive %u does not exist", i, prim[i]);
            pf[i] = prim[i];
        }
        if (kind == 4) pf[n + i] = face[i];
    }
    HIP_TRY(ctx, hipSetDevice(ctx->device));
    if (kind == 4) {
        std::vector<rt_mesh> meshes(ctx->meshes.n);
        HIP_TRY(ctx, hipMemcpy(meshes.data(), ctx->meshes.p, meshes.size() * sizeof(rt_mesh), hipMemcpyDeviceToHost));
        for (size_t i = 0; i < n; i++)
            if (face[i] >= meshes[prim[i]].face_count) return fail(ctx, RT_ERANGE, "unit probe %zu: face %u does not exist", i, face[i]);
    }
    std::vector<uint32_t> in(8 * n);
    memcpy(in.data(), rays, 6 * n * sizeof(float));
    memcpy(in.data() + 6 * n, pf.data(), 2 * n * sizeof(uint32_t));
    DeviceScene sc = device_scene(ctx);
    return debug_roundtrip(ctx, in.data(), in.size() * 4, out12, 12 * n * sizeof(float), [&](void *d_in, void *d_out) {
// ... 27 lines not shown
    if (n == 0) return RT_OK;
    HIP_TRY(ctx, hipSetDevice(ctx->device));
    return debug_roundtrip(ctx, in4, 4 * n * sizeof(float), out6, 6 * n * sizeof(float), [&](void *d_in, void *d_out) {
        return ctx->ks->launch_debug_div3(ctx, (const float *)d_in, (uint32_t)n, (float *)d_out);
    });
}

int rt_debug_queue_sums(rt_context *ctx, const float *in3, uint32_t npix, uint32_t count, uint32_t group_log2, float *out4) {
    if (!ctx || !in3 || !out4) return RT_EINVAL;
    if (npix < 1u || npix > 16u || count < 1u || npix * (uint64_t)count > 512u || group_log2 > 6u)
        return fail(ctx, RT_EINVAL, "queue_sums probe: %u pixels of %u samples do not fit one wave's queue", npix, count);
    HIP_TRY(ctx, hipSetDevice(ctx->device));
    return debug_roundtrip(ctx, in3, (size_t)npix * count * 3 * sizeof(float), out4, (size_t)npix * 4 * sizeof(float), [&](void *d_in, void *d_out) {
        return ctx->ks->launch_debug_queue_sums(ctx, (const float *)d_in, npix, count, group_log2, (float *)d_out);
    });
}

int rt_shard_slots(rt_context *ctx, int world, uint32_t *slots_out) {
    if (!ctx || !slots_out || world < 1) return RT_EINVAL;
    uint32_t tw = 1u << ctx->tile_w_log2, th = 1u << ctx->tile_h_log2;
    uint32_t tiles = ((ctx->width + tw - 1) / tw) * ((ctx->height + th - 1) / th);
    *slots_out = ((tiles + world - 1) / world) * tw * th;
    return RT_OK;
}

int rt_pack_accum(rt_context *ctx, void *d_packed, size_t bytes) {
    if (!ctx || !d_packed) return RT_EINVAL;
    uint32_t n = 0;
    rt_shard_slots(ctx, ctx->world, &n);
    if (bytes != (size_t)n * sizeof(float4)) return fail(ctx, RT_EINVAL, "packed buffer must be %zu bytes", (size_t)n * sizeof(float4));
    HIP_TRY(ctx, hipSetDevice(ctx->device));
    float cam0[12] = {0};
    FrameParams fp = frame_params(ctx, cam0, 0, 0, 0);
    hipLaunchKernelGGL(pt_pack, dim3((n + 255) / 256), dim3(256), 0, ctx->stream, fp, ctx->accum.p, (float4 *)d_packed, n);
    HIP_TRY(ctx, hipGetLastError());
    return RT_OK;
}

int rt_unpack_accum(rt_context *ctx, const void *d_packed, size_t bytes, int src_rank, int world) {
    if (!ctx || !d_packed) return RT_EINVAL;
    if (world < 1 || src_rank < 0 || src_rank >= world) return fail(ctx, RT_EINVAL, "rank %d of %d", src_rank, world);
    uint32_t n = 0;
    rt_shard_slots(ctx, world, &n);
    if (bytes != (size_t)n * sizeof(float4)) return fail(ctx, RT_EINVAL, "packed buffer must be %zu bytes", (size_t)n * sizeof(float4));
    HIP_TRY(ctx, hipSetDevice(ctx->device));
    float cam0[12] = {0};
    FrameParams fp = frame_params(ctx, cam0, 0, 0, 0, src_rank, world);
    if (fp.slot_end)
        hipLaunchKernelGGL(pt_unpack, dim3((fp.slot_end + 255) / 256), dim3(256), 0, ctx->stream, fp, (const float4 *)d_packed, ctx->accum.p);
    HIP_TRY(ctx, hipGetLastError());
    return RT_OK;
}

int rt_set_option(rt_context *ctx, int option, int value) {
    if (!ctx) return RT_EINVAL;
    ctx->prefix_changed();
    switch (option) {
        case RT_OPT_PREFIX_CACHE: ctx->prefix_cache.enabled = value != 0; return RT_OK;
        case RT_OPT_PREFIX_SHARING: ctx->prefix_sharing = value != 0; return RT_OK;
        case RT_OPT_SAMPLE_QUEUE: ctx->sample_queue = value != 0; return RT_OK;
        case RT_OPT_WALK_SLICES: ctx->walk_slices = value != 0; return RT_OK;
        case RT_OPT_WAVE_FILL: ctx->wave_fill = value != 0; return RT_OK;
        case RT_OPT_EXACT_GRID: ctx->sample_grid.exact = value != 0; return RT_OK;
        case RT_OPT_MOMENTS:
            if (value != 0 && value != 1) return fail(ctx, RT_EINVAL, "RT_OPT_MOMENTS takes 0 or 1");
            if (value == 1 && ctx->world > 1)
                return fail(ctx, RT_EINVAL, "sample moments on a sharded context (rank %d of %d)", ctx->rank, ctx->world);
            if ((value != 0) != ctx->moments.on) ctx->moments.valid = false;
            ctx->moments.on = value != 0;
            return RT_OK;
        case RT_OPT_LOOKAHEAD:
            if (value < 0 || value == 1 || value > RT_LOOKAHEAD_MAX) return fail(ctx, RT_EINVAL, "RT_OPT_LOOKAHEAD takes 0 or 2..%d", RT_LOOKAHEAD_MAX);
            ctx->lookahead.k = value;
            ctx->lookahead.ring_failed = false;
            return RT_OK;
        case RT_OPT_PREFIX_TREE:
            if (value < 0 || value > 2) return fail(ctx, RT_EINVAL, "RT_OPT_PREFIX_TREE takes 0, 1 or 2");
            ctx->prefix_tree = value;
            return RT_OK;
        case RT_OPT_ACCEL:
            if (value < 0 || value > 2) return fail(ctx, RT_EINVAL, "RT_OPT_ACCEL takes 0, 1 or 2");
            ctx->accel = value;
            return RT_OK;
        case RT_OPT_ARITH: {
            const KernelSet *ks = value == RT_ARITH_IEEE ? kernel_set_a0() : value == RT_ARITH_ROCM_OCL_NOCONTRACT ? kernel_set_a1()
                                  : value == RT_ARITH_ROCM_OCL ? kernel_set_a2() : nullptr;
            if (!ks) return fail(ctx, RT_EINVAL, "RT_OPT_ARITH takes RT_ARITH_IEEE (0), RT_ARITH_ROCM_OCL_NOCONTRACT (1) or RT_ARITH_ROCM_OCL (2)");
            HIP_TRY(ctx, hipSetDevice(ctx->device));
            HIP_TRY(ctx, hipStreamSynchronize(ctx->stream));
            ctx->arith = value;
            ctx->ks = ks;
            ctx->sample_counter = 0;
            return ctx->have_scene ? apply_arith(ctx) : RT_OK;
        }
        case RT_OPT_MAX_THREADS_PER_LAUNCH:
            if (value < 256) return fail(ctx, RT_EINVAL, "max threads per launch must be >= 256");
            ctx->max_threads_per_launch = (uint32_t)value;
            return RT_OK;
        default: return fail(ctx, RT_EINVAL, "unknown option %d", option);
    }
}

int rt_prefix_cache_stats(rt_context *ctx, uint64_t *hits, uint64_t *misses) {
    if (!ctx || !hits || !misses) return RT_EINVAL;
    *hits = ctx->prefix_cache.hits;
    *misses = ctx->prefix_cache.misses;
    return RT_OK;
}

int rt_sample_units(uint32_t seg_cap, uint32_t pixels_per_unit, uint32_t count_light, uint32_t count_heavy, uint32_t *units_out) {
    if (!units_out) return fail(nullptr, RT_EINVAL, "units_out is NULL");
    *units_out = 0;
    if (pixels_per_unit == 0) return fail(nullptr, RT_EINVAL, "pixels_per_unit is 0");
    const uint32_t cnt_l = std::min(count_light, seg_cap);
    const uint32_t cnt_h = std::min(count_heavy, seg_cap - cnt_l);
    const uint32_t units_h = cnt_h / pixels_per_unit + (cnt_h % pixels_per_unit != 0u);
    const uint32_t units_l = cnt_l / pixels_per_unit + (cnt_l % pixels_per_unit != 0u);
    *units_out = units_h + units_l;
    return RT_OK;
}

int rt_sample_grid_stats(rt_context *ctx, uint64_t *launches, uint64_t *exact, uint64_t *workgroups, uint64_t *live_last) {
    if (!ctx || !launches || !exact || !workgroups || !live_last) return RT_EINVAL;
    *launches = ctx->sample_grid.launches;
    *exact = ctx->sample_grid.exact_launches;
    *workgroups = ctx->sample_grid.workgroups;
    *live_last = ctx->sample_grid.live_last;
    return RT_OK;
}

int rt_debug_live_list(rt_context *ctx, uint32_t out[4]) {
    if (!ctx || !out) return RT_EINVAL;
    const rt_context::Slots &ss = ctx->slots;
    if (!ss.live.p || ctx->sample_grid.last_plan.pixels_per_wave == 0) return fail(ctx, RT_EINVAL, "no fused launch yet");
    HIP_TRY(ctx, hipSetDevice(ctx->device));
    uint32_t h[LIVE_COUNT_STRIDE];
    HIP_TRY(ctx, hipMemcpyAsync(h, ss.live.p + ss.capacity + 256u, sizeof h, hipMemcpyDeviceToHost, ctx->stream));
    HIP_TRY(ctx, hipStreamSynchronize(ctx->stream));
    out[0] = ctx->sample_grid.last_facts.seg_cap;
    out[1] = ctx->sample_grid.last_plan.pixels_per_wave;
    out[2] = h[0];
    out[3] = h[LIVE_HEAVY_COUNTER];
    return RT_OK;
}

int rt_debug_plan_samples(const rt_sample_facts *facts, rt_sample_plan *plan_out) {
    if (!facts || !plan_out || facts->count < 1u || facts->glog2 > 6u || facts->seg_cap < facts->n) return RT_EINVAL;
    *plan_out = pt::kernel_set_a2()->plan_samples(*facts);
    return RT_OK;
}

int rt_debug_last_sample_plan(rt_context *ctx, rt_sample_facts *facts_out, rt_sample_plan *plan_out) {
    if (!ctx || !facts_out || !plan_out) return RT_EINVAL;
    if (ctx->sample_grid.last_plan.pixels_per_wave == 0) return fail(ctx, RT_EINVAL, "no fused launch yet");
    *facts_out = ctx->sample_grid.last_facts;
    *plan_out = ctx->sample_grid.last_plan;
    return RT_OK;
}

int rt_debug_plan_camera_samples(const rt_camera_facts *facts, rt_camera_plan *plan_out) {
    if (!facts || !plan_out || facts->count < 1u || facts->count > RT_SPP_PER_LAUNCH || facts->glog2 > 6u) return RT_EINVAL;
    *plan_out = pt::kernel_set_a2()->plan_camera_samples(*facts);
    return RT_OK;
}

int rt_debug_last_camera_plan(rt_context *ctx, rt_camera_facts *facts_out, rt_camera_plan *plan_out) {
    if (!ctx || !facts_out || !plan_out) return RT_EINVAL;
    if (ctx->cameras.last_plan.block_size == 0) return fail(ctx, RT_EINVAL, "no camera launch yet");
    *facts_out = ctx->cameras.last_facts;
    *plan_out = ctx->cameras.last_plan;
    return RT_OK;
// ... 9 lines not shown

int rt_debug_queue_pixels(uint32_t count, uint32_t waves_per_simd, uint32_t static_float4, uint32_t granule, uint32_t *pixels_out) {
    if (!pixels_out || count < 1u || waves_per_simd < 1u || waves_per_simd > 8u || static_float4 > PT_LDS_STATIC_FLOAT4 ||
        (granule != 0u && (granule < 16u || granule > 8192u)))
        return RT_EINVAL;
    *pixels_out = pt::kernel_set_a2()->queue_pixels(count, waves_per_simd, static_float4, granule);
    return RT_OK;
}

int rt_debug_queue_occupancy(rt_context *ctx, uint32_t lds_bytes, int *blocks_out) {
    if (!ctx || !blocks_out) return RT_EINVAL;
    HIP_TRY(ctx, hipSetDevice(ctx->device));
    return ctx->ks->queue_occupancy(ctx, lds_bytes, blocks_out);
}

int rt_debug_wave_fixed(rt_context *ctx, uint64_t out[2]) {
    if (!ctx || !out) return RT_EINVAL;
    out[0] = ctx->sample_grid.count64_launches;
    out[1] = ctx->stage_block.builds;
    return RT_OK;
}

int rt_debug_stage_block(rt_context *ctx, float *out, size_t capacity_float4, uint32_t *float4_out) {
    if (!ctx || !float4_out) return RT_EINVAL;
    if (!ctx->have_scene || ctx->stage_block.generation != ctx->prefix_cache.generation)
        return fail(ctx, RT_EINVAL, "the staged scene block is not built (no fused launch since the last change)");
    const uint32_t n = lds_static_used((uint32_t)ctx->materials.n, (uint32_t)ctx->spheres.n, (uint32_t)ctx->planes.n);
    *float4_out = n;
    if (n == 0) return RT_OK;
    if (!out || capacity_float4 < n) return fail(ctx, RT_EINVAL, "the staged scene block holds %u float4", n);
    HIP_TRY(ctx, hipSetDevice(ctx->device));
    HIP_TRY(ctx, hipMemcpyAsync(out, reinterpret_cast<const char *>(ctx->materials.p) + stage_block_offset((uint32_t)ctx->materials.n),
                                n * sizeof(float4), hipMemcpyDeviceToHost, ctx->stream));
    HIP_TRY(ctx, hipStreamSynchronize(ctx->stream));
    return RT_OK;
}

int rt_reset_counters(rt_context *ctx) {
    if (!ctx) return RT_EINVAL;
    HIP_TRY(ctx, hipSetDevice(ctx->device));
    HIP_TRY(ctx, hipMemsetAsync(ctx->counters.p, 0, COUNTER_REPLICAS * COUNTER_STRIDE * sizeof(unsigned long long), ctx->stream));
    HIP_TRY(ctx, hipMemsetAsync(ctx->d_walk_overflow, 0, sizeof(uint32_t), ctx->stream));
    return RT_OK;
}

int rt_get_counters(rt_context *ctx, rt_counters *out) {
    if (!ctx || !out) return RT_EINVAL;
    HIP_TRY(ctx, hipSetDevice(ctx->device));
    std::vector<unsigned long long> h(COUNTER_REPLICAS * COUNTER_STRIDE);
    HIP_TRY(ctx, hipMemcpyAsync(h.data(), ctx->counters.p, h.size() * sizeof(unsigned long long), hipMemcpyDeviceToHost, ctx->stream));
    HIP_TRY(ctx, hipStreamSynchronize(ctx->stream));
    uint64_t *o = (uint64_t *)out;
    for (int i = 0; i < 14; i++) {
        o[i] = 0;
        for (int r = 0; r < COUNTER_REPLICAS; r++) o[i] += h[(size_t)r * COUNTER_STRIDE + i];
    }
    return RT_OK;
}

int rt_get_debug_counters(rt_context *ctx, uint64_t out[2]) {
    if (!ctx || !out) return RT_EINVAL;
    HIP_TRY(ctx, hipSetDevice(ctx->device));
    std::vector<unsigned long long> h(COUNTER_REPLICAS * COUNTER_STRIDE);
    HIP_TRY(ctx, hipMemcpyAsync(h.data(), ctx->counters.p, h.size() * sizeof(unsigned long long), hipMemcpyDeviceToHost, ctx->stream));
    HIP_TRY(ctx, hipStreamSynchronize(ctx->stream));
    out[0] = out[1] = 0;
    for (int r = 0; r < COUNTER_REPLICAS; r++) {
        out[0] += h[(size_t)r * COUNTER_STRIDE + 14];
        out[1] += h[(size_t)r * COUNTER_STRIDE + 15];
    }
#ifdef PT_WSTAT
    {
        unsigned long long v[12];
        if (hipMemcpy(v, ctx->counters.p + COUNTER_REPLICAS * COUNTER_STRIDE + 8, sizeof v, hipMemcpyDeviceToHost) == hipSuccess) {
            const char *names[12] = {"outer iterations", "active lanes", "phase-0 lanes", "phase-1 lanes", "phase-2 lanes", "walk slices",
                                     "walk steps", "node-test lanes", "(unused)", "leaf phases", "leaf lanes", "finished (idle) lanes"};
            for (int k = 0; k < 12; k++) fprintf(stderr, "[wstat] %-24s %llu\n", names[k], v[k]);
            (void)hipMemset(ctx->counters.p + COUNTER_REPLICAS * COUNTER_STRIDE + 8, 0, sizeof v);
        }
    }
#endif
#if PT_STAMPS
    {
        unsigned long long st[8];
        if (hipMemcpy(st, ctx->counters.p + COUNTER_REPLICAS * COUNTER_STRIDE, sizeof st, hipMemcpyDeviceToHost) == hipSuccess) {
            const char *names[6] = {"refill", "scatter", "hit:spheres", "hit:planes/lenses/models", "hit:rebuild+material", "loop"};
            double tot = 0;
            for (int k = 0; k < 6; k++) tot += (double)st[k];
            for (int k = 0; k < 6; k++) fprintf(stderr, "[stamps] %-26s %5.1f %%\n", names[k], tot > 0 ? 100.0 * st[k] / tot : 0.0);
        }
    }
#endif
    return RT_OK;
}

int rt_walk_overflow(rt_context *ctx, uint32_t *flags_out) {
    if (!ctx || !flags_out) return RT_EINVAL;
    HIP_TRY(ctx, hipSetDevice(ctx->device));
    HIP_TRY(ctx, hipMemcpyAsync(flags_out, ctx->d_walk_overflow, sizeof(uint32_t), hipMemcpyDeviceToHost, ctx->stream));
    HIP_TRY(ctx, hipStreamSynchronize(ctx->stream));
    return RT_OK;
}

int rt_debug_builtin(rt_context *ctx, int op, const float *in8, size_t n, float *out4) {
    if (!ctx || !in8 || !out4 || op < 0 || op > 12 || n > (1u << 26)) return RT_EINVAL;
    if (n == 0) return RT_OK;
    HIP_TRY(ctx, hipSetDevice(ctx->device));
    return debug_roundtrip(ctx, in8, 8 * n * sizeof(float), out4, 4 * n * sizeof(float), [&](void *d_in, void *d_out) {
        return ctx->ks->launch_debug_builtin(ctx, op, (const float *)d_in, (uint32_t)n, (float *)d_out);
    });
}

uint64_t rt_counters_bytes(const rt_counters *c) {
    if (!c) return 0;
    return 32 * c->t_sphere + 48 * c->t_plane + 64 * c->t_lens + 12 * c->t_model + 16 * c->t_mesh + 60 * c->t_tri +
           36 * c->h_tri + 48 * c->h_bounce + 12 * c->n_scatter + 4 * c->n_dielectric + 64 * c->n_texfetch +
           (48 + 16) * c->samples + 16 * c->image_reads;
}

int rt_kernel_ms_history(rt_context *ctx, float *ms, size_t cap, size_t *n_out) {
    if (!ctx || !ms || !n_out) return RT_EINVAL;
    HIP_TRY(ctx, hipSetDevice(ctx->device));
    size_t have = ctx->ev_count < (uint64_t)rt_context::EV_RING ? (size_t)ctx->ev_count : (size_t)rt_context::EV_RING;
    size_t n = have < cap ? have : cap;
    for (size_t i = 0; i < n; i++) {
        hipEvent_t *evp = ctx->ev[(ctx->ev_count - n + i) % rt_context::EV_RING];
        HIP_TRY(ctx, hipEventSynchronize(evp[1]));
        HIP_TRY(ctx, hipEventElapsedTime(&ms[i], evp[0], evp[1]));
    }
    *n_out = n;
    return RT_OK;
}

// ... 32 lines not shown
```

opencl-raytracing_amd/csrc/rt_context.hpp:

```cpp
#pragma once
#include <hip/hip_runtime.h>

#include <cstdarg>
#include <cstdint>
#include <cstring>
#include <string>
#include <utility>
#include <vector>

#include "pt_types.hpp"

template <class T>
struct DevBuf {
    T *p = nullptr;
    size_t n = 0;
    DevBuf() = default;
    DevBuf(const DevBuf &) = delete;
    DevBuf &operator=(const DevBuf &) = delete;
    DevBuf(DevBuf &&o) noexcept : p(o.p), n(o.n) { o.p = nullptr; o.n = 0; }
    DevBuf &operator=(DevBuf &&o) noexcept {
        std::swap(p, o.p);
        std::swap(n, o.n);
        return *this;
    }
// ... 115 lines not shown
        uint64_t exact_launches = 0;
        uint64_t workgroups = 0;
        uint64_t live_last = 0;
        rt_sample_facts last_facts = {};
        rt_sample_plan last_plan = {};
        uint64_t count64_launches = 0;
    } sample_grid;
    struct Lookahead {
        int k = 16;
        DevBuf<float4> ring;
        size_t ring_frames = 0;
        bool ring_failed = false;
        uint32_t pending = 0;
        uint32_t batch_frames = 0;
        uint32_t next_frame = 0;
        uint32_t next_sample = 0;
        uint64_t key_generation = 0, key_epoch = 0;
        uint32_t key_cam[12] = {};
        bool have_last_cam = false;
        uint32_t last_cam[12] = {};
        bool have_last_table = false;
        std::vector<uint32_t> last_table;
        bool key_is_table = false;
        uint64_t batches = 0, served = 0, direct = 0, discarded = 0;
    } lookahead;
    uint64_t image_epoch = 0;
    bool wave_fill = true;
    int prefix_tree = 1;
    bool prefix_sharing = true;
    bool sample_queue = true;
    DevBuf<uint2> walk_jobs;
    bool walk_slices = true;
    uint32_t accum_count = 0;
    uint32_t sample_counter = 0;
    bool count_enabled = false;

    struct Adaptive {
        DevBuf<float4> scratch;
        DevBuf<float4> half;
        DevBuf<uint32_t> block_active;
        DevBuf<float> block_err;
        DevBuf<unsigned long long> stats;
        DevBuf<float> m2_scratch;
        DevBuf<float> pixel_err;
        size_t block_capacity = 0;
        uint32_t blocks = 0;
        bool variance = false;
    } adaptive;
    struct Features {
        DevBuf<rt_feature> records;
        bool ready = false;
        DevBuf<float2> coverage;
        bool coverage_ready = false;
    } features;
    struct Denoise {
        DevBuf<float4> pingpong[2];
        DevBuf<float4> out;
        bool ready = false;
        DevBuf<float> var[2];
        bool var_ready = false;
    } denoise;

    struct Moments {
        bool on = false;
        bool valid = false;
        DevBuf<float> m2;
// ... 2 lines not shown

    struct Cameras {
        static constexpr uint32_t RING = 4;
        DevBuf<float> table;
        float *h_table = nullptr;
        hipEvent_t read[RING] = {};
        uint64_t launches = 0;
        rt_camera_facts last_facts = {};
        rt_camera_plan last_plan = {};
    } cameras;

    struct Rays {
        DevBuf<rt_ray> buf;
        size_t count = 0;
        rt_camera_facts last_facts = {};
        rt_camera_plan last_plan = {};
    } rays;

    int rank = 0, world = 1, tile_w_log2 = 3, tile_h_log2 = 3;
    uint32_t max_threads_per_launch = 1u << 30;
};

namespace rtamd {
using namespace pt;

int fail(rt_context *ctx, int code, const char *fmt, ...);
int read_back(rt_context *ctx, void *dst, size_t bytes, const void *src, size_t need, const char *what, bool ready = true,
              const char *producer = nullptr);

#define HIP_TRY(ctx, expr)                                                                        \
    do {                                                                                          \
        hipError_t e_ = (expr);                                                                   \
        if (e_ != hipSuccess) return fail(ctx, RT_EHIP, "%s: %s", #expr, hipGetErrorString(e_)); \
    } while (0)

inline DeviceScene device_scene(const rt_context *ctx) {
    DeviceScene s;
    s.materials = ctx->materials.p;
    s.spheres = ctx->spheres.p;
    s.sph4 = ctx->sph4.p;
    s.sphere_batches = ctx->sphere_batches;
    s.material_count = (uint32_t)ctx->materials.n;
    s.faces = ctx->faces.p;
    s.mesh_face_base = ctx->mesh_face_base.p;
    s.mbvh_nodes = ctx->mbvh_nodes.p;
    s.mbvh_faces = ctx->mbvh_faces.p;
    s.mbvh_face_idx = ctx->mbvh_face_idx.p;
    s.mesh_bvh_root = (ctx->have_mesh_bvh && ctx->accel != 0) ? ctx->mesh_bvh_root.p : nullptr;
    bool use_bvh = ctx->bvh_node_count && (ctx->accel == 2 || (ctx->accel == 1 && ctx->spheres.n >= ACCEL_MIN_SPHERES));
    s.bvh_nodes = ctx->bvh_nodes.p;
    s.bvh_sph = ctx->bvh_sph.p;
    s.bvh_idx = ctx->bvh_idx.p;
    s.bvh_links = ctx->bvh_links.p;
    s.bvh_node_count = use_bvh ? ctx->bvh_node_count : 0;
    for (int k = 0; k < 3; k++) { s.bvh_lo[k] = ctx->bvh_lo[k]; s.bvh_hi[k] = ctx->bvh_hi[k]; }
    s.bvh_rmax = ctx->bvh_rmax;
    s.walk_overflow = ctx->d_walk_overflow;
    s.planes = ctx->planes.p;
    s.lenses = ctx->lenses.p;
    s.vertices = ctx->vertices.p;
    s.uvs = ctx->uvs.p;
    s.indices = ctx->indices.p;
    s.meshes = ctx->meshes.p;
    s.models = ctx->models.p;
    s.table = ctx->table.p;
    s.tex = ctx->tex.p;
// ... 13 lines not shown
    uint32_t tiles_x, tiles_total, owned_tiles, slots;
};
inline Shard shard_of(const rt_context *ctx, int rank, int world) {
    Shard s;
    uint32_t tw = 1u << ctx->tile_w_log2, th = 1u << ctx->tile_h_log2;
    s.tiles_x = (ctx->width + tw - 1) / tw;
    uint32_t tiles_y = (ctx->height + th - 1) / th;
    s.tiles_total = s.tiles_x * tiles_y;
    s.owned_tiles = s.tiles_total > (uint32_t)rank ? (s.tiles_total - rank + world - 1) / world : 0;
    s.slots = s.owned_tiles * tw * th;
    return s;
}

inline FrameParams frame_params(const rt_context *ctx, const float cam[12], uint32_t first, uint32_t count, uint32_t glog2,
                         int rank = -1, int world = 1) {
    if (rank < 0) { rank = ctx->rank; world = ctx->world; }
    FrameParams fp;
    memcpy(fp.cam, cam, sizeof fp.cam);
    Shard sh = shard_of(ctx, rank, world);
    fp.w = ctx->width;
    fp.h = ctx->height;
    fp.tile_w_log2 = ctx->tile_w_log2;
    fp.tile_h_log2 = ctx->tile_h_log2;
    fp.tiles_x = sh.tiles_x;
    fp.tiles_total = sh.tiles_total;
    fp.rank = (uint32_t)rank;
    fp.world = (uint32_t)world;
    fp.slot_begin = 0;
    fp.slot_end = sh.slots;
    fp.first = first;
    fp.count = count;
    fp.group_log2 = glog2;
    fp.seg_cap = 0;
    fp.trees = nullptr;
    fp.tree_wait = nullptr;
    fp.tree_count = nullptr;
    fp.tree_cap = 0;
    fp.lds_face_f4 = 0;
    fp.block_active = nullptr;
    fp.blk_w_log2 = fp.blk_h_log2 = 0;
    fp.blocks_x = 0;
    fp.la_ring = nullptr;
    fp.la_image = nullptr;
    fp.m2 = nullptr;
    {
        volatile float c = (float)count;
        volatile float q = 1.0f / c;
        fp.inv_count = count ? q : 0.0f;
    }
    return fp;
}

inline void apply_mask(FrameParams &fp, const BlockMask *mask) {
    if (!mask) return;
    fp.block_active = mask->active;
    fp.blk_w_log2 = mask->w_log2;
    fp.blk_h_log2 = mask->h_log2;
    fp.blocks_x = mask->blocks_x;
}

inline bool scene_has_accel(const DeviceScene &sc) { return sc.bvh_node_count != 0 || sc.mesh_bvh_root != nullptr; }

inline int ensure_slots(rt_context *ctx, size_t slots) {
    rt_context::Slots &s = ctx->slots;
    if (slots <= s.capacity) return RT_OK;
    s = {};
// ... 113 lines not shown
```

opencl-raytracing_amd/csrc/rt_denoise.hip:

```cpp
#include <hip/hip_runtime.h>

#include <algorithm>
#include <cfloat>
#include <cmath>

#include "rt_context.hpp"

using namespace rtamd;


#define PT_DN_TILE 16
#define PT_DN_SIDE (PT_DN_TILE + 4)
#define PT_DN_POINTS (PT_DN_SIDE * PT_DN_SIDE)
#define PT_DN_OFF 0xFFFFFFFEu
#define PT_DN_XCDS 8u
struct DenoiseStep {
    uint32_t w, h;
    uint32_t step_log2;
    uint32_t tiles_x;
    uint32_t groups;
    float inv_n, inv_x, inv_a;
    uint32_t split;
    uint32_t first, last;
    float inv_c;
// ... 284 lines not shown
    StepPlan sp = {};
    DenoiseStep &ds = sp.ds;
    ds.w = (uint32_t)ctx->width;
    ds.h = (uint32_t)ctx->height;
    ds.step_log2 = i;
    const uint32_t s = 1u << i;
    const uint32_t lat_w = (ds.w + s - 1u) >> i, lat_h = (ds.h + s - 1u) >> i;
    ds.tiles_x = (lat_w + PT_DN_TILE - 1u) / PT_DN_TILE;
    const uint32_t tiles_y = (lat_h + PT_DN_TILE - 1u) / PT_DN_TILE;
    ds.groups = s * s * ds.tiles_x * tiles_y;
    ds.inv_n = inv_sq(p.sigma_normal);
    ds.inv_x = inv_sq(p.sigma_position);
    ds.inv_a = inv_sq(p.sigma_albedo);
    ds.split = (p.flags & RT_DENOISE_SPLIT_OBJECTS) ? 1u : 0u;
    ds.first = i == 0;
    ds.last = i + 1 == p.iterations;
    sp.grid = (ds.groups + PT_DN_XCDS - 1u) / PT_DN_XCDS * PT_DN_XCDS;
    sp.src = i == 0 ? ctx->accum.p : d.pingpong[(i - 1) & 1u].p;
    sp.dst = ds.last ? d.out.p : d.pingpong[i & 1u].p;
    return sp;
}

const float4 *guide(const rt_context *ctx) { return reinterpret_cast<const float4 *>(ctx->features.records.p); }

int denoise_variance(rt_context *ctx, const rt_denoise_variance_params *vp, bool measured) {
    const Params p = vp ? Params{vp->iterations, vp->sigma_luminance, vp->sigma_normal, vp->sigma_position, vp->sigma_albedo, vp->flags}
                        : Params{};
    int rc = validate(ctx, vp != nullptr, p);
    if (rc) return rc;
    if (measured && !ctx->moments.target())
        return fail(ctx, RT_ESTATE, "the sample moments are not valid: set RT_OPT_MOMENTS to 1, then rt_clear or rt_render_adaptive");
    HIP_TRY(ctx, hipSetDevice(ctx->device));
    if ((rc = ensure_buffers(ctx, true)) != RT_OK) return rc;
    rt_context::Denoise &d = ctx->denoise;
    const uint32_t w = (uint32_t)ctx->width, h = (uint32_t)ctx->height;
    DenoiseVariance dv;
    dv.w = w;
    dv.h = h;
    dv.tiles_x = (w + PT_DN_TILE - 1u) / PT_DN_TILE;
    dv.inv_n = inv_sq(p.sigma_normal);
    dv.inv_x = inv_sq(p.sigma_position);
    dv.inv_a = inv_sq(p.sigma_albedo);
    dv.split = (p.flags & RT_DENOISE_SPLIT_OBJECTS) ? 1u : 0u;
    const bool chains = (p.flags & RT_DENOISE_SPLIT_CHAINS) != 0;
    hipLaunchKernelGGL(chains ? pt_dn_variance_ch : pt_dn_variance, dim3(dv.tiles_x * ((h + PT_DN_TILE - 1u) / PT_DN_TILE)), dim3(256),
                       0, ctx->stream, dv, ctx->accum.p, guide(ctx), d.var[0].p);
    HIP_TRY(ctx, hipGetLastError());
    if (measured) {
        hipLaunchKernelGGL(pt_dn_measured, dim3((w * h + 255u) / 256u), dim3(256), 0, ctx->stream, ctx->accum.p, ctx->moments.m2.p,
                           d.var[0].p, w * h);
        HIP_TRY(ctx, hipGetLastError());
    }
    for (uint32_t i = 0; i < p.iterations; i++) {
        StepPlan sp = plan_step(ctx, p, i);
        sp.ds.lum_on = std::isinf(p.sigma_own) ? 0u : 1u;
        sp.ds.sigma_l = sp.ds.lum_on ? p.sigma_own : 0.0f;
        hipLaunchKernelGGL(chains ? pt_atrous_vg_ch : pt_atrous_vg, dim3(sp.grid), dim3(256), 0, ctx->stream, sp.ds, sp.src, d.var[0].p, ctx->accum.p,
                           guide(ctx), sp.dst, d.var[1].p);
        HIP_TRY(ctx, hipGetLastError());
    }
    d.ready = true;
    d.var_ready = true;
    return RT_OK;
}

}


extern "C" {

int rt_denoise(rt_context *ctx, const rt_denoise_params *dp) {
    const Params p = dp ? Params{dp->iterations, dp->sigma_color, dp->sigma_normal, dp->sigma_position, dp->sigma_albedo, dp->flags}
                        : Params{};
    int rc = validate(ctx, dp != nullptr, p);
    if (rc) return rc;
    HIP_TRY(ctx, hipSetDevice(ctx->device));
    if ((rc = ensure_buffers(ctx, false)) != RT_OK) return rc;
    for (uint32_t i = 0; i < p.iterations; i++) {
        StepPlan sp = plan_step(ctx, p, i);
        sp.ds.inv_c = inv_sq(p.sigma_own, (int)i);
        hipLaunchKernelGGL((p.flags & RT_DENOISE_SPLIT_CHAINS) ? pt_atrous_ch : pt_atrous, dim3(sp.grid), dim3(256), 0, ctx->stream, sp.ds, sp.src, guide(ctx), sp.dst);
        HIP_TRY(ctx, hipGetLastError());
    }
    ctx->denoise.ready = true;
    return RT_OK;
}

int rt_read_denoised(rt_context *ctx, float *rgba, size_t bytes) {
    if (!ctx) return RT_EINVAL;
    const rt_context::Denoise &d = ctx->denoise;
    return read_back(ctx, rgba, bytes, d.out.p, (size_t)ctx->width * ctx->height * sizeof(float4), "image", d.ready, "rt_denoise");
}

int rt_device_denoised(rt_context *ctx, void **d_rgba) {
    if (!ctx || !d_rgba) return RT_EINVAL;
    if (!ctx->denoise.ready) return fail(ctx, RT_ESTATE, "no rt_denoise call since the frame was (re)allocated");
    *d_rgba = ctx->denoise.out.p;
    return RT_OK;
}

int rt_denoise_variance(rt_context *ctx, const rt_denoise_variance_params *p) { return denoise_variance(ctx, p, false); }
int rt_denoise_moments(rt_context *ctx, const rt_denoise_variance_params *p) { return denoise_variance(ctx, p, true); }

int rt_read_variance(rt_context *ctx, int which, float *out, size_t bytes) {
    if (!ctx) return RT_EINVAL;
    if (which < 0 || which > 1) return fail(ctx, RT_EINVAL, "variance buffer %d outside 0..1", which);
    const rt_context::Denoise &d = ctx->denoise;
    return read_back(ctx, out, bytes, d.var[which].p, (size_t)ctx->width * ctx->height * sizeof(float), "variance", d.var_ready,
                     "rt_denoise_variance");
}
// ... 11 lines not shown
```

opencl-raytracing_amd/raytracer.py:

```python
import ctypes as C
import os

import numpy as np

from . import _abi
from .scene import SceneCreator

_HERE = os.path.dirname(os.path.abspath(__file__))
LIB_PATH = os.path.join(_HERE, "librt_amd.so")

SYMBOLS = (
    "rt_abi_version", "rt_last_error", "rt_create", "rt_destroy", "rt_resize", "rt_set_stream", "rt_set_scene",
    "rt_set_textures", "rt_set_seed", "rt_set_random_table", "rt_get_random_table", "rt_make_random_table",
    "rt_set_shard", "rt_render", "rt_render_again", "rt_sample_counter", "rt_clear", "rt_render_spp", "rt_resolve",
    "rt_sync", "rt_trace_samples", "rt_read_image", "rt_read_linear", "rt_device_image", "rt_device_accum",
    "rt_enable_counters", "rt_reset_counters", "rt_get_counters", "rt_counters_bytes", "rt_last_kernel_ms",
    "rt_kernel_ms_history", "rt_stage_ms_history", "rt_debug_hit", "rt_debug_material", "rt_debug_div3", "rt_device_info", "rt_set_option", "rt_shard_slots", "rt_pack_accum", "rt_unpack_accum",
    "rt_get_debug_counters", "rt_debug_check_accel", "rt_walk_overflow", "rt_debug_builtin",
    "rt_render_adaptive", "rt_read_sample_counts", "rt_read_block_error",
    "rt_render_features", "rt_read_features", "rt_device_features", "rt_render_features_chain", "rt_feature_chain_signature",
    "rt_denoise", "rt_read_denoised", "rt_device_denoised",
    "rt_denoise_variance", "rt_read_variance", "rt_device_variance",
    "rt_read_moments", "rt_device_moments", "rt_moments_merge", "rt_denoise_moments",
    "rt_prefix_cache_stats", "rt_lookahead_stats", "rt_lookahead_plan",
    "rt_sample_units", "rt_sample_grid_stats", "rt_debug_live_list", "rt_debug_wave_fixed", "rt_debug_stage_block", "rt_debug_queue_pixels", "rt_debug_queue_occupancy", "rt_debug_queue_sums",
    "rt_debug_plan_samples", "rt_debug_last_sample_plan",
    "rt_render_spp_cameras", "rt_debug_plan_camera_samples", "rt_debug_last_camera_plan",
    "rt_render_features_cameras", "rt_read_feature_coverage", "rt_device_feature_coverage", "rt_debug_plan_feature_cameras",
    "rt_render_adaptive_cameras", "rt_render_again_cameras",
    "rt_render_adaptive_variance", "rt_render_adaptive_variance_cameras", "rt_read_pixel_error", "rt_device_pixel_error",
    "rt_upload_rays", "rt_device_rays", "rt_render_rays", "rt_render_features_rays", "rt_debug_last_ray_plan",
    "rt_render_ray_sets",
    "rt_render_adaptive_rays", "rt_render_adaptive_variance_rays",
    "rt_intersect_rays", "rt_occluded_rays", "rt_device_alloc", "rt_device_free", "rt_device_copy",
    "rt_occluded_hemispheres", "rt_render_hemispheres",
)

OPT_PREFIX_SHARING, OPT_MAX_THREADS_PER_LAUNCH, OPT_SAMPLE_QUEUE, OPT_ACCEL, OPT_WALK_SLICES, OPT_ARITH, OPT_PREFIX_TREE, OPT_WAVE_FILL = 1, 2, 3, 4, 5, 6, 7, 8
OPT_PREFIX_CACHE = 9
OPT_LOOKAHEAD = 10
OPT_EXACT_GRID = 11
OPT_MOMENTS = 12
ARITH_IEEE, ARITH_ROCM_OCL_NOCONTRACT, ARITH_ROCM_OCL = 0, 1, 2
FOLLOW_REFLECTIVE, FOLLOW_REFRACTIVE, FOLLOW_DIELECTRIC = _abi.FOLLOW_REFLECTIVE, _abi.FOLLOW_REFRACTIVE, _abi.FOLLOW_DIELECTRIC
FOLLOW_ALL = FOLLOW_REFLECTIVE | FOLLOW_REFRACTIVE | FOLLOW_DIELECTRIC
ARITH_NAMES = {"ieee": ARITH_IEEE, "rocm-opencl-nocontract": ARITH_ROCM_OCL_NOCONTRACT, "rocm-opencl": ARITH_ROCM_OCL}


class RtError(RuntimeError):
    def __init__(self, code, msg):
        super().__init__("librt_amd: %s (code %d)" % (msg, code))
        self.code = code


_lib = None


def load_library(path=LIB_PATH):
    global _lib
    if _lib is not None:
        return _lib
    if not os.path.isfile(path):
        raise OSError("%s not found — the HIP library is not built (run __graft_entry__.build()); "
                      "there is no CPU fallback" % path)
    try:
        import torch
    except ImportError:
        pass
    lib = C.CDLL(path)
    for s in SYMBOLS:
        getattr(lib, s)
    vp, u32, u64, sz, fp = C.c_void_p, C.c_uint32, C.c_uint64, C.c_size_t, C.POINTER(C.c_float)
    lib.rt_last_error.restype = C.c_char_p
    lib.rt_last_error.argtypes = [vp]
    lib.rt_create.argtypes = [C.c_int, C.c_int, C.c_int, C.POINTER(vp)]
# ... 205 lines not shown
        try:
            self.close()
        except Exception:
            pass

    def setScene(self, scene):
        self.scene = scene
        d = scene.desc()
        self._check(self._lib.rt_set_scene(self._ctx, C.byref(d)))
        tex, tw, th, layers = scene.texture_args()
        self._check(self._lib.rt_set_textures(self._ctx, tex, tw, th, layers))

    def setSeed(self, seed):
        self._check(self._lib.rt_set_seed(self._ctx, seed))

    def setRandomTable(self, table):
        table = np.ascontiguousarray(table, dtype=np.float32)
        self._check(self._lib.rt_set_random_table(self._ctx, table.ctypes.data, table.size))

    def getRandomTable(self):
        out = np.empty(_abi.RANDOM_TABLE_FLOATS, dtype=np.float32)
        self._check(self._lib.rt_get_random_table(self._ctx, out.ctypes.data, out.size))
        return out

    def setShard(self, rank, world, tile_w=8, tile_h=8):
        self._check(self._lib.rt_set_shard(self._ctx, rank, world, tile_w, tile_h))
        self._world = int(world)

    OPT_PREFIX_SHARING, OPT_MAX_THREADS_PER_LAUNCH, OPT_SAMPLE_QUEUE, OPT_ACCEL, OPT_WALK_SLICES, OPT_ARITH, OPT_PREFIX_TREE, OPT_WAVE_FILL = 1, 2, 3, 4, 5, 6, 7, 8
    OPT_PREFIX_CACHE = 9
    OPT_LOOKAHEAD = 10
    OPT_EXACT_GRID = 11
    OPT_MOMENTS = 12

    def setOption(self, option, value):
        self._check(self._lib.rt_set_option(self._ctx, option, int(value)))

    def shardSlots(self, world):
        n = C.c_uint32()
        self._check(self._lib.rt_shard_slots(self._ctx, world, C.byref(n)))
        return n.value

    def packAccum(self, device_ptr, nbytes):
        self._check(self._lib.rt_pack_accum(self._ctx, C.c_void_p(device_ptr), nbytes))

    def unpackAccum(self, device_ptr, nbytes, src_rank, world):
        self._check(self._lib.rt_unpack_accum(self._ctx, C.c_void_p(device_ptr), nbytes, src_rank, world))

    def setStream(self, hip_stream):
        self._check(self._lib.rt_set_stream(self._ctx, C.c_void_p(hip_stream or 0)))

    def resize(self, w, h):
        self._check(self._lib.rt_resize(self._ctx, w, h))
        self.width, self.height = w, h

    def setTime(self, time):
        """Declared, never defined in the reference (include/raytracer.h:45); a stub."""

    def render(self, camera):
        self._check(self._lib.rt_render(self._ctx, _cam_block(camera).ctypes.data))

    def renderAgain(self, camera):
        self._check(self._lib.rt_render_again(self._ctx, _cam_block(camera).ctypes.data))

    def renderAgainCameras(self, blocks):
        blocks = _cam_blocks(blocks)
# ... 436 lines not shown
        return DeviceBuffer(p.value, self.height, self.width, self)

    def deviceAccum(self):
        p = C.c_void_p()
        self._check(self._lib.rt_device_accum(self._ctx, C.byref(p)))
        return DeviceBuffer(p.value, self.height, self.width, self)

    def enableCounters(self, on=True):
        self._check(self._lib.rt_enable_counters(self._ctx, 1 if on else 0))

    def resetCounters(self):
        self._check(self._lib.rt_reset_counters(self._ctx))

    def counters(self):
        c = _abi.Counters()
        self._check(self._lib.rt_get_counters(self._ctx, C.byref(c)))
        return c

    def debugCounters(self):
        out = (C.c_uint64 * 2)()
        self._check(self._lib.rt_get_debug_counters(self._ctx, out))
        return int(out[0]), int(out[1])

    def walkOverflow(self):
        out = C.c_uint32()
        self._check(self._lib.rt_walk_overflow(self._ctx, C.byref(out)))
        return int(out.value)

    def prefixCacheStats(self):
        hits, misses = C.c_uint64(), C.c_uint64()
        self._check(self._lib.rt_prefix_cache_stats(self._ctx, C.byref(hits), C.byref(misses)))
        return int(hits.value), int(misses.value)

    def lookaheadStats(self):
        v = [C.c_uint64() for _ in range(4)]
        self._check(self._lib.rt_lookahead_stats(self._ctx, *[C.byref(x) for x in v]))
        return tuple(int(x.value) for x in v)

    lookaheadPlan = staticmethod(lookahead_plan)

    def sampleGridStats(self):
        v = [C.c_uint64() for _ in range(4)]
        self._check(self._lib.rt_sample_grid_stats(self._ctx, *[C.byref(x) for x in v]))
        return tuple(int(x.value) for x in v)

    sampleUnits = staticmethod(sample_units)

    def liveList(self):
        out = (C.c_uint32 * 4)()
        self._check(self._lib.rt_debug_live_list(self._ctx, out))
        return tuple(int(v) for v in out)

    def waveFixedStats(self):
        out = (C.c_uint64 * 2)()
        self._check(self._lib.rt_debug_wave_fixed(self._ctx, out))
        return tuple(int(v) for v in out)

    planSamples = staticmethod(plan_samples)
    planCameraSamples = staticmethod(plan_camera_samples)
    planFeatureCameras = staticmethod(plan_feature_cameras)

    def lastSamplePlan(self):
        f, p = _abi.SampleFacts(), _abi.SamplePlan()
        self._check(self._lib.rt_debug_last_sample_plan(self._ctx, C.byref(f), C.byref(p)))
        return f.as_dict(), p.as_dict()

# ... 75 lines not shown
```

Measured before the change: 145,400.

## Defer accumulator clear and overwrite it in the first fused sample launch

rt_clear no longer memsets the float4 accumulator. It marks a pending clear, and the first qualifying single-range queue launch (64 spp, no moments, mask or accel) writes sums directly instead of read-modify-write. Every other consumer materialises the memset first through new CLEAR_TRY/SYNC_TRY wrappers. This removes a full-frame memset plus one accumulator read per frame, and adds 32-bit pixel addressing and a paired LDS load in the tree reduction. The cost is state-tracking complexity, with the risk of a missed materialisation leaving stale data.

```diff
diff --git a/include/rt_amd.h b/include/rt_amd.h
--- a/include/rt_amd.h
+++ b/include/rt_amd.h
@@ -346,6 +346,7 @@
 #define RT_OPT_LOOKAHEAD 10
 #define RT_OPT_EXACT_GRID 11
 #define RT_OPT_MOMENTS 12
+#define RT_OPT_ACCUM_STORE 13
 #define RT_OPT_ARITH 6
 #define RT_ARITH_IEEE 0
 #define RT_ARITH_ROCM_OCL_NOCONTRACT 1
@@ -379,6 +380,8 @@
 int rt_stage_ms_history(rt_context *ctx, float *first_ms, float *second_ms, size_t cap, size_t *n_out);
 
 int rt_prefix_cache_stats(rt_context *ctx, uint64_t *hits, uint64_t *misses);
+
+int rt_accum_store_stats(rt_context *ctx, uint64_t *stored, uint64_t *materialised);
 
 int rt_lookahead_stats(rt_context *ctx, uint64_t *batches, uint64_t *served, uint64_t *direct, uint64_t *discarded);
 
diff --git a/opencl-raytracing_amd/_abi.py b/opencl-raytracing_amd/_abi.py
--- a/opencl-raytracing_amd/_abi.py
+++ b/opencl-raytracing_amd/_abi.py
@@ -174,6 +174,7 @@
 
 def prefix_cache_prototypes(lib):
     lib.rt_prefix_cache_stats.argtypes = [C.c_void_p, C.POINTER(C.c_uint64), C.POINTER(C.c_uint64)]
+    lib.rt_accum_store_stats.argtypes = [C.c_void_p, C.POINTER(C.c_uint64), C.POINTER(C.c_uint64)]
 
 
 def lookahead_prototypes(lib):
diff --git a/opencl-raytracing_amd/csrc/pt_kernels.hip b/opencl-raytracing_amd/csrc/pt_kernels.hip
--- a/opencl-raytracing_amd/csrc/pt_kernels.hip
+++ b/opencl-raytracing_amd/csrc/pt_kernels.hip
@@ -68,6 +68,16 @@
     a.z += sum.z;
     a.w += (float)count;
     accum[pix] = a;
+}
+#ifndef PT_ACCUM_STORE
+#define PT_ACCUM_STORE 1
+#endif
+PT_DEV void accumulate_store(float4 *__restrict__ accum, size_t pix, V3 sum, uint32_t count) {
+    accum[pix] = make_float4(0.0f + sum.x, 0.0f + sum.y, 0.0f + sum.z, 0.0f + (float)count);
+}
+PT_DEV void accumulate_any(const FrameParams &fp, float4 *__restrict__ accum, size_t pix, V3 sum, uint32_t count) {
+    if (PT_ACCUM_STORE && fp.store) accumulate_store(accum, pix, sum, count);
+    else accumulate(accum, pix, sum, count);
 }
 
 PT_DEV void moments_update(const float4 *accum, float *m2, size_t pix, V3 sum, uint32_t count, float m2B) {
@@ -312,7 +322,8 @@
             if (accum) {
                 const V3 fsum = final_sum(xyz(rec.out), fp.count, fp.group_log2);
                 if (fp.m2) moments_update(accum, fp.m2, (size_t)y * fp.w + x, fsum, fp.count, 0.0f);
-                accumulate(accum, (size_t)y * fp.w + x, fsum, fp.count);
+                if (COUNT || ACCEL) accumulate(accum, (size_t)y * fp.w + x, fsum, fp.count);
+                else accumulate_any(fp, accum, (size_t)y * fp.w + x, fsum, fp.count);
             }
             if (COUNT) cn.c[CN_SAMPLES] += 1;
         } else {
@@ -406,7 +417,7 @@
     if (!slot_to_pixel(fp, e.slot, x, y)) return;
     const V3 fsum = final_sum(mk(e.r, e.g, e.b), fp.count, fp.group_log2);
     if (fp.m2) moments_update(accum, fp.m2, (size_t)y * fp.w + x, fsum, fp.count, 0.0f);
-    accumulate(accum, (size_t)y * fp.w + x, fsum, fp.count);
+    accumulate_any(fp, accum, (size_t)y * fp.w + x, fsum, fp.count);
 }
 #endif
 
@@ -687,21 +698,44 @@
     }
     return sum;
 }
-template <int CL = -1>
+#ifndef PT_SUMS_ADDR
+#define PT_SUMS_ADDR 1
+#endif
+static_assert((uint64_t)RT_MAX_DIM * RT_MAX_DIM <= 0xFFFFFFFFull, "a pixel index fits 32 bits (queue_sums_tree, PT_SUMS_ADDR)");
+PT_DEV V3 queue_lane_pair64(LdsF32 sl, bool owned) {
+    V3 sum = mk(0.0f, 0.0f, 0.0f);
+    if (owned) {
+        sum = sum + mk(sl[0], sl[1], sl[2]);
+        sum = sum + (mk(0.0f, 0.0f, 0.0f) + mk(sl[96], sl[97], sl[98]));
+    }
+    return sum;
+}
+template <int CL = -1, bool STORE = false>
 PT_DEV void queue_sums_tree(const WaveQueue &q, const FrameParams &fp, float4 *__restrict__ accum) {
     if (CL == 6) {
         static_assert(QUEUE_SLOTS / 64u <= 8u, "two passes of four pixels");
         const uint32_t lane = threadIdx.x, half = lane >> 5, i = lane & 31u, row = lane >> 4;
+        const LdsF32 sl0 = q.slot + 3u * (half * 64u + i);
 #pragma unroll
         for (uint32_t pb = 0; pb < 8u; pb += 4u) {
             if (pb >= q.npix) break;
-            V3 a = queue_lane_slot64(q, pb + half, i), b = queue_lane_slot64(q, pb + 2u + half, i);
-            a = a + queue_lane_slot64(q, pb + half, i + 32u);
-            b = b + queue_lane_slot64(q, pb + 2u + half, i + 32u);
+            V3 a, b;
+            if (STORE && PT_SUMS_ADDR) {
+                a = queue_lane_pair64(sl0 + 3u * 64u * pb, pb + half < q.npix);
+                b = queue_lane_pair64(sl0 + 3u * 64u * (pb + 2u), pb + 2u + half < q.npix);
+            } else {
+                a = queue_lane_slot64(q, pb + half, i), b = queue_lane_slot64(q, pb + 2u + half, i);
+                a = a + queue_lane_slot64(q, pb + half, i + 32u);
+                b = b + queue_lane_slot64(q, pb + 2u + half, i + 32u);
+            }
             V3 sum = mk(row_pair_add(a.x, b.x), row_pair_add(a.y, b.y), row_pair_add(a.z, b.z));
             sum = row_add<1>(row_add<2>(row_add<4>(row_add<8>(sum))));
             const uint32_t p = pb + ((row & 1u) << 1 | row >> 1);
-            if (p < q.npix && (lane & 15u) == 0u) accumulate(accum, (size_t)q.xy[p].y * fp.w + q.xy[p].x, sum, 64u);
+            if (p < q.npix && (lane & 15u) == 0u) {
+                if (STORE && PT_SUMS_ADDR) accumulate_any(fp, accum, q.xy[p].y * (uint32_t)fp.w + q.xy[p].x, sum, 64u);
+                else if (STORE) accumulate_any(fp, accum, (size_t)q.xy[p].y * fp.w + q.xy[p].x, sum, 64u);
+                else accumulate(accum, (size_t)q.xy[p].y * fp.w + q.xy[p].x, sum, 64u);
+            }
         }
         return;
     }
@@ -732,11 +766,11 @@
         }
     }
 }
-template <bool MOMENTS, bool BUTTERFLY = false, int CL = -1>
+template <bool MOMENTS, bool BUTTERFLY = false, int CL = -1, bool STORE = false>
 PT_DEV void queue_sums(const WaveQueue &q, const FrameParams &fp, float4 *__restrict__ accum) {
     __builtin_amdgcn_fence(__ATOMIC_SEQ_CST, "wavefront");
     __builtin_amdgcn_wave_barrier();
-    if (PT_QUEUE_SUMS_TREE && !MOMENTS && !BUTTERFLY) return queue_sums_tree<CL>(q, fp, accum);
+    if (PT_QUEUE_SUMS_TREE && !MOMENTS && !BUTTERFLY) return queue_sums_tree<CL, STORE>(q, fp, accum);
     const uint32_t lane = threadIdx.x;
     const uint32_t g = 1u << fp.group_log2, ppp = 64u >> fp.group_log2;
     for (uint32_t pb = 0; pb < q.npix; pb += ppp) {
@@ -1645,6 +1679,7 @@
 int launch_render(rt_context *ctx, int mode, const float cam[12], uint32_t first, uint32_t count, uint32_t glog2, float4 *accum,
                   const BlockMask *mask, float *m2) {
     if (mode < MODE_ACCUM || mode > MODE_RETRACE) return fail(ctx, RT_EINVAL, "unknown render mode %d", mode);
+    CLEAR_TRY(ctx);
     FrameParams fp = frame_params(ctx, cam, first, count, glog2);
     apply_mask(fp, mask);
     fp.m2 = mode == MODE_ACCUM ? m2 : nullptr;
@@ -1851,6 +1886,17 @@
     ctx->stage_block.builds++;
 }
 
+static bool accum_store_may_qualify(const rt_context *ctx, const FrameParams &fp, const float4 *accum, const BlockMask *mask,
+                                    const float4 *ring, const float *m2, bool one_range) {
+    return PT_ACCUM_STORE && ctx->accum_store && ctx->clear_pending && accum && accum == ctx->accum.p && !ring && !mask && !m2 &&
+           one_range && fp.world == 1u && !ctx->count_enabled && fp.count == 64u && fp.group_log2 == 6u;
+}
+static bool accum_store_qualifies(const rt_context *ctx, const FrameParams &fp, const SamplePlan &plan, const float4 *accum,
+                                  const BlockMask *mask, const float4 *ring, const float *m2, bool one_range) {
+    return accum_store_may_qualify(ctx, fp, accum, mask, ring, m2, one_range) && plan.family == RT_PLAN_QUEUE && !plan.accel &&
+           !plan.count && !plan.moments && plan.geom < 2u && plan.count_log2 == 6u && plan.waves == PT_Q_WAVES;
+}
+
 static int launch_fused_any(rt_context *ctx, const float cam[12], uint32_t first, uint32_t count, uint32_t glog2, float4 *accum,
                             const BlockMask *mask, float4 *ring, float *m2) {
     FrameParams fp = frame_params(ctx, cam, first, count, glog2);
@@ -1879,6 +1925,7 @@
     bool exact = false;
     if ((rc = learn_live_counts(ctx, hit, live_count, &exact)) != RT_OK) return rc;
     rt_context::SampleGrid &sg = ctx->sample_grid;
+    if (!accum_store_may_qualify(ctx, fp, accum, mask, ring, m2, per >= slots) && (rc = materialise_clear(ctx)) != RT_OK) return rc;
     hipEvent_t *evp = ctx->ev[ctx->ev_count % rt_context::EV_RING];
     HIP_TRY(ctx, hipEventRecord(evp[0], ctx->stream));
     for (uint32_t b = 0; b < slots; b = fp.slot_end) {
@@ -1893,9 +1940,14 @@
         const SampleFacts facts = sample_facts(ctx, sc, fp, exact);
         const SamplePlan plan = plan_samples(facts);
         fp.lds_face_f4 = plan.lds_face_f4;
+        const bool store = accum_store_qualifies(ctx, fp, plan, accum, mask, ring, m2, per >= slots);
+        if (store) fp.store = 1u;
+        else if ((rc = materialise_clear(ctx)) != RT_OK) return rc;
         launch_first_stage(ctx, sc, fp, hit, ring != nullptr, accum, live_count);
         HIP_TRY(ctx, hipEventRecord(evp[2], ctx->stream));
         if ((rc = launch_plan(ctx, plan, sc, fp, accum, live_count)) != RT_OK) return rc;
+        if (store) ctx->clear_pending = false, ctx->clears_stored++;
+        fp.store = 0u;
         sg.last_facts = facts, sg.last_plan = plan;
         sg.launches++;
         sg.workgroups += plan.grid_units;
@@ -1963,6 +2015,7 @@
         if (mask && src.n != (size_t)ctx->width * ctx->height)
             return fail(ctx, RT_EINVAL, "a masked ray launch takes one ray per pixel of the %d x %d frame", ctx->width, ctx->height);
     }
+    CLEAR_TRY(ctx);
     FrameParams fp = src.rays ? frame_params(ctx, src.cam0, first, count, glog2, 0, 1)
                               : frame_params(ctx, src.cam0, first, count, glog2);
     apply_mask(fp, mask);
diff --git a/opencl-raytracing_amd/csrc/pt_samples_q_kernel.hpp b/opencl-raytracing_amd/csrc/pt_samples_q_kernel.hpp
--- a/opencl-raytracing_amd/csrc/pt_samples_q_kernel.hpp
+++ b/opencl-raytracing_amd/csrc/pt_samples_q_kernel.hpp
@@ -237,6 +237,6 @@
     static_assert(!CAM_LA || (CAM && ACCEL), "the look-ahead kernels of the camera entry's ACCEL rows");
     constexpr bool LA_BRANCH = CAM ? !ACCEL : !COUNT && !MOMENTS;
     if (CAM_LA || (!RAYS && LA_BRANCH && fp.la_ring)) queue_replay<CAM>(q, fp);
-    else queue_sums<MOMENTS, COUNT || ACCEL, COUNT_LOG2>(q, fp, accum);
+    else queue_sums<MOMENTS, COUNT || ACCEL, COUNT_LOG2, PT_Q_LOOKAHEAD_FORM == 0 && !COUNT && !ACCEL && !MOMENTS && !CAM && COUNT_LOG2 == 6>(q, fp, accum);
     flush_counters<COUNT>(cn, counters, 1);
 }
diff --git a/opencl-raytracing_amd/csrc/pt_types.hpp b/opencl-raytracing_amd/csrc/pt_types.hpp
--- a/opencl-raytracing_amd/csrc/pt_types.hpp
+++ b/opencl-raytracing_amd/csrc/pt_types.hpp
@@ -1,5 +1,6 @@
 #pragma once
 #include <hip/hip_runtime.h>
+#include <stddef.h>
 #include <stdint.h>
 
 #include "../../include/rt_amd.h"
@@ -117,6 +118,7 @@
     uint32_t group_log2;
     uint32_t seg_cap;
     float inv_count;
+    uint32_t store;
     PixelTree *trees;
     PixelRec *tree_wait;
     uint32_t *tree_count;
@@ -133,6 +135,7 @@
     };
     float *m2;
 };
+static_assert(sizeof(FrameParams) == 192 && offsetof(FrameParams, trees) == 112, "FrameParams::store fills padding: no field moves");
 
 struct BlockMask {
     const uint32_t *active;
diff --git a/opencl-raytracing_amd/csrc/rt_amd.hip b/opencl-raytracing_amd/csrc/rt_amd.hip
--- a/opencl-raytracing_amd/csrc/rt_amd.hip
+++ b/opencl-raytracing_amd/csrc/rt_amd.hip
@@ -292,6 +292,7 @@
     ctx->width = w;
     ctx->height = h;
     ctx->accum_count = 0;
+    ctx->clear_pending = false;
     ctx->sample_counter = 0;
     return RT_OK;
 }
@@ -314,8 +315,9 @@
     if (!dst || bytes != need) return fail(ctx, RT_EINVAL, "%s buffer must be %zu bytes", what, need);
     if (!ready) return fail(ctx, RT_ESTATE, "no %s call since the frame was (re)allocated", producer);
     HIP_TRY(ctx, hipSetDevice(ctx->device));
+    CLEAR_TRY(ctx);
     HIP_TRY(ctx, hipMemcpyAsync(dst, src, need, hipMemcpyDeviceToHost, ctx->stream));
-    HIP_TRY(ctx, hipStreamSynchronize(ctx->stream));
+    SYNC_TRY(ctx);
     return RT_OK;
 }
 }
@@ -345,7 +347,7 @@
         int rc = ctx->ks->launch_face_normals(ctx, ctx->faces.p, (uint32_t)(ctx->h_faces.size() / 3));
         if (rc == RT_OK) rc = ctx->ks->launch_face_normals(ctx, ctx->mbvh_faces.p, (uint32_t)(ctx->h_mbvh_faces.size() / 3));
         if (rc != RT_OK) return rc;
-        HIP_TRY(ctx, hipStreamSynchronize(ctx->stream));
+        SYNC_TRY(ctx);
     }
     return RT_OK;
 }
@@ -442,14 +444,14 @@
     if (width < 1 || height < 1 || width > RT_MAX_DIM || height > RT_MAX_DIM)
         return fail(ctx, RT_EINVAL, "frame size %dx%d outside 1..%d", width, height, RT_MAX_DIM);
     HIP_TRY(ctx, hipSetDevice(ctx->device));
-    HIP_TRY(ctx, hipStreamSynchronize(ctx->stream));
+    SYNC_TRY(ctx);
     return alloc_frame(ctx, width, height);
 }
 
 int rt_set_stream(rt_context *ctx, void *hip_stream) {
     if (!ctx) return RT_EINVAL;
     HIP_TRY(ctx, hipSetDevice(ctx->device));
-    HIP_TRY(ctx, hipStreamSynchronize(ctx->stream));
+    SYNC_TRY(ctx);
     ctx->stream = hip_stream ? (hipStream_t)hip_stream : ctx->own_stream;
     ctx->prefix_changed();
     ctx->ev_count = 0;
@@ -465,7 +467,7 @@
         std::string err;
         if (int rc = prepare_scene(*d, ps, err)) return fail(ctx, rc, "%s", err.c_str());
         HIP_TRY(ctx, hipSetDevice(ctx->device));
-        HIP_TRY(ctx, hipStreamSynchronize(ctx->stream));
+        SYNC_TRY(ctx);
         ctx->have_scene = false;
         HIP_TRY(ctx, ctx->materials.upload(d->materials, d->material_count,
                                            lds_static_used(d->material_count, d->sphere_count, d->plane_count) * sizeof(float4)));
@@ -514,7 +516,7 @@
     if (!ctx) return RT_EINVAL;
     ctx->prefix_changed();
     HIP_TRY(ctx, hipSetDevice(ctx->device));
-    HIP_TRY(ctx, hipStreamSynchronize(ctx->stream));
+    SYNC_TRY(ctx);
     if (layers == 0) {
         float4 zero = make_float4(0.0f, 0.0f, 0.0f, 0.0f);
         HIP_TRY(ctx, ctx->tex.upload(&zero, 1));
@@ -536,7 +538,7 @@
     if (!table || n != RT_RANDOM_TABLE_FLOATS) return fail(ctx, RT_EINVAL, "table must hold %d floats", RT_RANDOM_TABLE_FLOATS);
     ctx->prefix_changed();
     HIP_TRY(ctx, hipSetDevice(ctx->device));
-    HIP_TRY(ctx, hipStreamSynchronize(ctx->stream));
+    SYNC_TRY(ctx);
     HIP_TRY(ctx, ctx->table.upload(table, n));
     return RT_OK;
 }
@@ -552,7 +554,7 @@
     if (!ctx) return RT_EINVAL;
     if (!out || n != RT_RANDOM_TABLE_FLOATS) return fail(ctx, RT_EINVAL, "table must hold %d floats", RT_RANDOM_TABLE_FLOATS);
     HIP_TRY(ctx, hipSetDevice(ctx->device));
-    HIP_TRY(ctx, hipStreamSynchronize(ctx->stream));
+    SYNC_TRY(ctx);
     HIP_TRY(ctx, hipMemcpy(out, ctx->table.p, n * sizeof(float), hipMemcpyDeviceToHost));
     return RT_OK;
 }
@@ -657,7 +659,7 @@
     la.next_sample++;
     la.served++;
     ctx->sample_counter++;
-    HIP_TRY(ctx, hipStreamSynchronize(ctx->stream));
+    SYNC_TRY(ctx);
     return RT_OK;
 }
 
@@ -699,7 +701,7 @@
     remember_camera(ctx, camera);
     ctx->sample_counter = 0;
     if ((rc = ctx->ks->launch_render(ctx, MODE_TRACE, camera, 0, 1, 0, ctx->accum.p, nullptr, nullptr)) != RT_OK) return rc;
-    HIP_TRY(ctx, hipStreamSynchronize(ctx->stream));
+    SYNC_TRY(ctx);
     return RT_OK;
 }
 
@@ -730,7 +732,7 @@
     la.direct++;
     ctx->sample_counter++;
     if ((rc = ctx->ks->launch_render(ctx, MODE_RETRACE, camera, ctx->sample_counter, 1, 0, ctx->accum.p, nullptr, nullptr)) != RT_OK) return rc;
-    HIP_TRY(ctx, hipStreamSynchronize(ctx->stream));
+    SYNC_TRY(ctx);
     return RT_OK;
 }
 
@@ -774,7 +776,9 @@
 int rt_clear(rt_context *ctx) {
     if (!ctx) return RT_EINVAL;
     HIP_TRY(ctx, hipSetDevice(ctx->device));
-    HIP_TRY(ctx, hipMemsetAsync(ctx->accum.p, 0, (size_t)ctx->width * ctx->height * sizeof(float4), ctx->stream));
+    CLEAR_TRY(ctx);
+    if (ctx->accum_store) ctx->clear_pending = true;
+    else HIP_TRY(ctx, hipMemsetAsync(ctx->accum.p, 0, (size_t)ctx->width * ctx->height * sizeof(float4), ctx->stream));
     ctx->accum_count = 0;
     return moments_begin(ctx);
 }
@@ -991,12 +995,13 @@
     la.direct++;
     ctx->sample_counter++;
     if ((rc = ctx->ks->launch_render(ctx, MODE_RETRACE, cameras + 12u * (size_t)(s % n_cameras), ctx->sample_counter, 1, 0, ctx->accum.p, nullptr, nullptr)) != RT_OK) return rc;
-    HIP_TRY(ctx, hipStreamSynchronize(ctx->stream));
+    SYNC_TRY(ctx);
     return RT_OK;
 }
 
 static int resolve_into(rt_context *ctx, int linear_only) {
     uint32_t n = (uint32_t)ctx->width * ctx->height;
+    CLEAR_TRY(ctx);
     hipLaunchKernelGGL(pt_resolve, dim3((n + 255) / 256), dim3(256), 0, ctx->stream, ctx->accum.p, ctx->image.p, n,
                        linear_only);
     HIP_TRY(ctx, hipGetLastError());
@@ -1084,6 +1089,7 @@
     if (mom && !a.m2_scratch.p) HIP_TRY(ctx, a.m2_scratch.alloc(px));
     ctx->image_epoch++;
     const size_t bytes = px * sizeof(float4);
+    ctx->clear_pending = false;
     HIP_TRY(ctx, hipMemsetAsync(ctx->accum.p, 0, bytes, ctx->stream));
     HIP_TRY(ctx, hipMemsetAsync(a.scratch.p, 0, bytes, ctx->stream));
     if (rule == RULE_DAMMERTZ) HIP_TRY(ctx, hipMemsetAsync(a.half.p, 0, bytes, ctx->stream));
@@ -1127,7 +1133,7 @@
         rounds++;
         ctx->accum_count = first + c;
         HIP_TRY(ctx, hipMemcpyAsync(st.data(), a.stats.p, st_bytes, hipMemcpyDeviceToHost, ctx->stream));
-        HIP_TRY(ctx, hipStreamSynchronize(ctx->stream));
+        SYNC_TRY(ctx);
         uint64_t still = 0;
         for (uint32_t r = 0; r < PT_MERGE_REPLICAS; r++) {
             still += st[r * PT_MERGE_STRIDE];
@@ -1137,7 +1143,7 @@
         if (still == 0) break;
     }
     if ((rc = resolve_into(ctx, 0)) != RT_OK) return rc;
-    HIP_TRY(ctx, hipStreamSynchronize(ctx->stream));
+    SYNC_TRY(ctx);
     a.blocks = blocks;
     a.variance = rule == RULE_VARIANCE;
     out->rounds = rounds;
@@ -1233,8 +1239,9 @@
     if (!counts || bytes != n * sizeof(uint32_t)) return fail(ctx, RT_EINVAL, "count buffer must be %zu bytes", n * sizeof(uint32_t));
     HIP_TRY(ctx, hipSetDevice(ctx->device));
     std::vector<float4> h(n);
+    CLEAR_TRY(ctx);
     HIP_TRY(ctx, hipMemcpyAsync(h.data(), ctx->accum.p, n * sizeof(float4), hipMemcpyDeviceToHost, ctx->stream));
-    HIP_TRY(ctx, hipStreamSynchronize(ctx->stream));
+    SYNC_TRY(ctx);
     for (size_t i = 0; i < n; i++) counts[i] = (uint32_t)h[i].w;
     return RT_OK;
 }
@@ -1444,7 +1451,7 @@
     if (bytes == 0) return RT_OK;
     HIP_TRY(ctx, hipSetDevice(ctx->device));
     HIP_TRY(ctx, hipMemcpyAsync(dst, src, bytes, to_device ? hipMemcpyHostToDevice : hipMemcpyDeviceToHost, ctx->stream));
-    HIP_TRY(ctx, hipStreamSynchronize(ctx->stream));
+    SYNC_TRY(ctx);
     return RT_OK;
 }
 
@@ -1551,7 +1558,7 @@
 int rt_sync(rt_context *ctx) {
     if (!ctx) return RT_EINVAL;
     HIP_TRY(ctx, hipSetDevice(ctx->device));
-    HIP_TRY(ctx, hipStreamSynchronize(ctx->stream));
+    SYNC_TRY(ctx);
     return RT_OK;
 }
 
@@ -1575,7 +1582,7 @@
     const FrameParams fp = frame_params(ctx, camera, 0, 1, 0);
     if ((rc = ctx->ks->launch_probe(ctx, fp, device_scene(ctx), d_in.p, (uint32_t)n, d_out.p)) != RT_OK) return rc;
     HIP_TRY(ctx, hipMemcpyAsync(out_rgb, d_out.p, 3 * n * sizeof(float), hipMemcpyDeviceToHost, ctx->stream));
-    HIP_TRY(ctx, hipStreamSynchronize(ctx->stream));
+    SYNC_TRY(ctx);
     return RT_OK;
 }
 
@@ -1591,10 +1598,11 @@
     HIP_TRY(ctx, hipSetDevice(ctx->device));
     DevBuf<float4> tmp;
     HIP_TRY(ctx, tmp.alloc(n));
+    CLEAR_TRY(ctx);
     hipLaunchKernelGGL(pt_resolve, dim3((n + 255) / 256), dim3(256), 0, ctx->stream, ctx->accum.p, tmp.p, (uint32_t)n, 1);
     HIP_TRY(ctx, hipGetLastError());
     HIP_TRY(ctx, hipMemcpyAsync(rgba, tmp.p, bytes, hipMemcpyDeviceToHost, ctx->stream));
-    HIP_TRY(ctx, hipStreamSynchronize(ctx->stream));
+    SYNC_TRY(ctx);
     return RT_OK;
 }
 
@@ -1606,6 +1614,8 @@
 
 int rt_device_accum(rt_context *ctx, void **d_rgba) {
     if (!ctx || !d_rgba) return RT_EINVAL;
+    HIP_TRY(ctx, hipSetDevice(ctx->device));
+    CLEAR_TRY(ctx);
     *d_rgba = ctx->accum.p;
     return RT_OK;
 }
@@ -1638,7 +1648,7 @@
     HIP_TRY(ctx, hipMemcpyAsync(d_in.p, in, bytes, hipMemcpyHostToDevice, ctx->stream));
     if (int rc = launch(d_in.p, d_out.p)) return rc;
     HIP_TRY(ctx, hipMemcpyAsync(out, d_out.p, out_bytes, hipMemcpyDeviceToHost, ctx->stream));
-    HIP_TRY(ctx, hipStreamSynchronize(ctx->stream));
+    SYNC_TRY(ctx);
     return RT_OK;
 }
 }
@@ -1732,6 +1742,7 @@
     HIP_TRY(ctx, hipSetDevice(ctx->device));
     float cam0[12] = {0};
     FrameParams fp = frame_params(ctx, cam0, 0, 0, 0);
+    CLEAR_TRY(ctx);
     hipLaunchKernelGGL(pt_pack, dim3((n + 255) / 256), dim3(256), 0, ctx->stream, fp, ctx->accum.p, (float4 *)d_packed, n);
     HIP_TRY(ctx, hipGetLastError());
     return RT_OK;
@@ -1746,6 +1757,7 @@
     HIP_TRY(ctx, hipSetDevice(ctx->device));
     float cam0[12] = {0};
     FrameParams fp = frame_params(ctx, cam0, 0, 0, 0, src_rank, world);
+    CLEAR_TRY(ctx);
     if (fp.slot_end)
         hipLaunchKernelGGL(pt_unpack, dim3((fp.slot_end + 255) / 256), dim3(256), 0, ctx->stream, fp, (const float4 *)d_packed, ctx->accum.p);
     HIP_TRY(ctx, hipGetLastError());
@@ -1762,6 +1774,14 @@
         case RT_OPT_WALK_SLICES: ctx->walk_slices = value != 0; return RT_OK;
         case RT_OPT_WAVE_FILL: ctx->wave_fill = value != 0; return RT_OK;
         case RT_OPT_EXACT_GRID: ctx->sample_grid.exact = value != 0; return RT_OK;
+        case RT_OPT_ACCUM_STORE:
+            if (value != 0 && value != 1) return fail(ctx, RT_EINVAL, "RT_OPT_ACCUM_STORE takes 0 or 1");
+            if (value == 0) {
+                HIP_TRY(ctx, hipSetDevice(ctx->device));
+                CLEAR_TRY(ctx);
+            }
+            ctx->accum_store = value != 0;
+            return RT_OK;
         case RT_OPT_MOMENTS:
             if (value != 0 && value != 1) return fail(ctx, RT_EINVAL, "RT_OPT_MOMENTS takes 0 or 1");
             if (value == 1 && ctx->world > 1)
@@ -1787,7 +1807,7 @@
                                   : value == RT_ARITH_ROCM_OCL ? kernel_set_a2() : nullptr;
             if (!ks) return fail(ctx, RT_EINVAL, "RT_OPT_ARITH takes RT_ARITH_IEEE (0), RT_ARITH_ROCM_OCL_NOCONTRACT (1) or RT_ARITH_ROCM_OCL (2)");
             HIP_TRY(ctx, hipSetDevice(ctx->device));
-            HIP_TRY(ctx, hipStreamSynchronize(ctx->stream));
+            SYNC_TRY(ctx);
             ctx->arith = value;
             ctx->ks = ks;
             ctx->sample_counter = 0;
@@ -1801,6 +1821,13 @@
     }
 }
 
+int rt_accum_store_stats(rt_context *ctx, uint64_t *stored, uint64_t *materialised) {
+    if (!ctx || !stored || !materialised) return RT_EINVAL;
+    *stored = ctx->clears_stored;
+    *materialised = ctx->clears_materialised;
+    return RT_OK;
+}
+
 int rt_prefix_cache_stats(rt_context *ctx, uint64_t *hits, uint64_t *misses) {
     if (!ctx || !hits || !misses) return RT_EINVAL;
     *hits = ctx->prefix_cache.hits;
@@ -1836,7 +1863,7 @@
     HIP_TRY(ctx, hipSetDevice(ctx->device));
     uint32_t h[LIVE_COUNT_STRIDE];
     HIP_TRY(ctx, hipMemcpyAsync(h, ss.live.p + ss.capacity + 256u, sizeof h, hipMemcpyDeviceToHost, ctx->stream));
-    HIP_TRY(ctx, hipStreamSynchronize(ctx->stream));
+    SYNC_TRY(ctx);
     out[0] = ctx->sample_grid.last_facts.seg_cap;
     out[1] = ctx->sample_grid.last_plan.pixels_per_wave;
     out[2] = h[0];
@@ -1912,7 +1939,7 @@
     HIP_TRY(ctx, hipSetDevice(ctx->device));
     HIP_TRY(ctx, hipMemcpyAsync(out, reinterpret_cast<const char *>(ctx->materials.p) + stage_block_offset((uint32_t)ctx->materials.n),
                                 n * sizeof(float4), hipMemcpyDeviceToHost, ctx->stream));
-    HIP_TRY(ctx, hipStreamSynchronize(ctx->stream));
+    SYNC_TRY(ctx);
     return RT_OK;
 }
 
@@ -1929,7 +1956,7 @@
     HIP_TRY(ctx, hipSetDevice(ctx->device));
     std::vector<unsigned long long> h(COUNTER_REPLICAS * COUNTER_STRIDE);
     HIP_TRY(ctx, hipMemcpyAsync(h.data(), ctx->counters.p, h.size() * sizeof(unsigned long long), hipMemcpyDeviceToHost, ctx->stream));
-    HIP_TRY(ctx, hipStreamSynchronize(ctx->stream));
+    SYNC_TRY(ctx);
     uint64_t *o = (uint64_t *)out;
     for (int i = 0; i < 14; i++) {
         o[i] = 0;
@@ -1943,7 +1970,7 @@
     HIP_TRY(ctx, hipSetDevice(ctx->device));
     std::vector<unsigned long long> h(COUNTER_REPLICAS * COUNTER_STRIDE);
     HIP_TRY(ctx, hipMemcpyAsync(h.data(), ctx->counters.p, h.size() * sizeof(unsigned long long), hipMemcpyDeviceToHost, ctx->stream));
-    HIP_TRY(ctx, hipStreamSynchronize(ctx->stream));
+    SYNC_TRY(ctx);
     out[0] = out[1] = 0;
     for (int r = 0; r < COUNTER_REPLICAS; r++) {
         out[0] += h[(size_t)r * COUNTER_STRIDE + 14];
@@ -1978,7 +2005,7 @@
     if (!ctx || !flags_out) return RT_EINVAL;
     HIP_TRY(ctx, hipSetDevice(ctx->device));
     HIP_TRY(ctx, hipMemcpyAsync(flags_out, ctx->d_walk_overflow, sizeof(uint32_t), hipMemcpyDeviceToHost, ctx->stream));
-    HIP_TRY(ctx, hipStreamSynchronize(ctx->stream));
+    SYNC_TRY(ctx);
     return RT_OK;
 }
 
diff --git a/opencl-raytracing_amd/csrc/rt_context.hpp b/opencl-raytracing_amd/csrc/rt_context.hpp
--- a/opencl-raytracing_amd/csrc/rt_context.hpp
+++ b/opencl-raytracing_amd/csrc/rt_context.hpp
@@ -171,6 +171,9 @@
     DevBuf<uint2> walk_jobs;
     bool walk_slices = true;
     uint32_t accum_count = 0;
+    bool accum_store = true;
+    bool clear_pending = false;
+    uint64_t clears_stored = 0, clears_materialised = 0;
     uint32_t sample_counter = 0;
     bool count_enabled = false;
 
@@ -239,6 +242,30 @@
     do {                                                                                          \
         hipError_t e_ = (expr);                                                                   \
         if (e_ != hipSuccess) return fail(ctx, RT_EHIP, "%s: %s", #expr, hipGetErrorString(e_)); \
+    } while (0)
+
+inline int materialise_clear(rt_context *ctx) {
+    if (!ctx->clear_pending) return RT_OK;
+    HIP_TRY(ctx, hipMemsetAsync(ctx->accum.p, 0, (size_t)ctx->width * ctx->height * sizeof(float4), ctx->stream));
+    ctx->clear_pending = false;
+    ctx->clears_materialised++;
+    return RT_OK;
+}
+inline int sync_stream(rt_context *ctx) {
+    const int rc = materialise_clear(ctx);
+    if (rc != RT_OK) return rc;
+    HIP_TRY(ctx, hipStreamSynchronize(ctx->stream));
+    return RT_OK;
+}
+#define SYNC_TRY(ctx)                         \
+    do {                                      \
+        const int rc_ = sync_stream(ctx);     \
+        if (rc_ != RT_OK) return rc_;         \
+    } while (0)
+#define CLEAR_TRY(ctx)                        \
+    do {                                      \
+        const int rc_ = materialise_clear(ctx); \
+        if (rc_ != RT_OK) return rc_;         \
     } while (0)
 
 inline DeviceScene device_scene(const rt_context *ctx) {
@@ -318,6 +345,7 @@
     fp.count = count;
     fp.group_log2 = glog2;
     fp.seg_cap = 0;
+    fp.store = 0;
     fp.trees = nullptr;
     fp.tree_wait = nullptr;
     fp.tree_count = nullptr;
diff --git a/opencl-raytracing_amd/csrc/rt_denoise.hip b/opencl-raytracing_amd/csrc/rt_denoise.hip
--- a/opencl-raytracing_amd/csrc/rt_denoise.hip
+++ b/opencl-raytracing_amd/csrc/rt_denoise.hip
@@ -340,6 +340,7 @@
         return fail(ctx, RT_ESTATE, "the sample moments are not valid: set RT_OPT_MOMENTS to 1, then rt_clear or rt_render_adaptive");
     HIP_TRY(ctx, hipSetDevice(ctx->device));
     if ((rc = ensure_buffers(ctx, true)) != RT_OK) return rc;
+    CLEAR_TRY(ctx);
     rt_context::Denoise &d = ctx->denoise;
     const uint32_t w = (uint32_t)ctx->width, h = (uint32_t)ctx->height;
     DenoiseVariance dv;
@@ -384,6 +385,7 @@
     if (rc) return rc;
     HIP_TRY(ctx, hipSetDevice(ctx->device));
     if ((rc = ensure_buffers(ctx, false)) != RT_OK) return rc;
+    CLEAR_TRY(ctx);
     for (uint32_t i = 0; i < p.iterations; i++) {
         StepPlan sp = plan_step(ctx, p, i);
         sp.ds.inv_c = inv_sq(p.sigma_own, (int)i);
diff --git a/opencl-raytracing_amd/raytracer.py b/opencl-raytracing_amd/raytracer.py
--- a/opencl-raytracing_amd/raytracer.py
+++ b/opencl-raytracing_amd/raytracer.py
@@ -22,7 +22,7 @@
     "rt_denoise", "rt_read_denoised", "rt_device_denoised",
     "rt_denoise_variance", "rt_read_variance", "rt_device_variance",
     "rt_read_moments", "rt_device_moments", "rt_moments_merge", "rt_denoise_moments",
-    "rt_prefix_cache_stats", "rt_lookahead_stats", "rt_lookahead_plan",
+    "rt_prefix_cache_stats", "rt_accum_store_stats", "rt_lookahead_stats", "rt_lookahead_plan",
     "rt_sample_units", "rt_sample_grid_stats", "rt_debug_live_list", "rt_debug_wave_fixed", "rt_debug_stage_block", "rt_debug_queue_pixels", "rt_debug_queue_occupancy", "rt_debug_queue_sums",
     "rt_debug_plan_samples", "rt_debug_last_sample_plan",
     "rt_render_spp_cameras", "rt_debug_plan_camera_samples", "rt_debug_last_camera_plan",
@@ -41,6 +41,7 @@
 OPT_LOOKAHEAD = 10
 OPT_EXACT_GRID = 11
 OPT_MOMENTS = 12
+OPT_ACCUM_STORE = 13
 ARITH_IEEE, ARITH_ROCM_OCL_NOCONTRACT, ARITH_ROCM_OCL = 0, 1, 2
 FOLLOW_REFLECTIVE, FOLLOW_REFRACTIVE, FOLLOW_DIELECTRIC = _abi.FOLLOW_REFLECTIVE, _abi.FOLLOW_REFRACTIVE, _abi.FOLLOW_DIELECTRIC
 FOLLOW_ALL = FOLLOW_REFLECTIVE | FOLLOW_REFRACTIVE | FOLLOW_DIELECTRIC
@@ -312,6 +313,7 @@
     OPT_LOOKAHEAD = 10
     OPT_EXACT_GRID = 11
     OPT_MOMENTS = 12
+    OPT_ACCUM_STORE = 13
 
     def setOption(self, option, value):
         self._check(self._lib.rt_set_option(self._ctx, option, int(value)))
@@ -814,6 +816,11 @@
         self._check(self._lib.rt_prefix_cache_stats(self._ctx, C.byref(hits), C.byref(misses)))
         return int(hits.value), int(misses.value)
 
+    def accumStoreStats(self):
+        stored, mat = C.c_uint64(), C.c_uint64()
+        self._check(self._lib.rt_accum_store_stats(self._ctx, C.byref(stored), C.byref(mat)))
+        return int(stored.value), int(mat.value)
+
     def lookaheadStats(self):
         v = [C.c_uint64() for _ in range(4)]
         self._check(self._lib.rt_lookahead_stats(self._ctx, *[C.byref(x) for x in v]))
```

Result: faster. 148,200 (median of 6 runs) (+1.9%).
